# lucidrains/audiolm-pytorch

Measured on AMD Instinct MI355X. Metric: audio-tokens/sec fwd+bwd, CoarseTransformer d=1024 seq=2048, higher is better.
Workload: dtype bf16; 1 GPU; CoarseTransformer dim=1024 depth=6 heads=8 (MQA) num_coarse_quantizers=3 codebook=1024 semantic=500 residual_streams=4 flash_attn=True; per-GPU B=8, N=2048 (509 semantic + 512x3 coarse ids + eos/start); mask_prob=0.15; global_batch=8, seq_len=2048, parallelism=dp1, schedule=one hipGraph replay per step (captured fwd + bwd)

## Files before the change

audiolm-pytorch_amd/_lib.py:

```python
from __future__ import annotations

import ctypes
import os
from ctypes import c_float, c_int, c_longlong, c_ulonglong, c_void_p

_HERE = os.path.dirname(os.path.abspath(__file__))
LIB_PATH = os.environ.get('ALM_LIB_PATH') or os.path.join(_HERE, 'libaudiolm_hip.so')

_P, _I, _L, _F, _U = c_void_p, c_int, c_longlong, c_float, c_ulonglong

SIGNATURES = {
    'alm_gemm_bf16_nt': [_P, _P, _P, _P, _I, _I, _I, _L, _L, _L, _I, _I, _L, _L, _L, _L, _L, _L, _F, _I, _I, _P],
    'alm_gemm_bf16_nt_ws': [_P, _P, _P, _P, _I, _I, _I, _L, _L, _L, _I, _I, _L, _L, _L, _L, _L, _L, _F, _I, _I, _P, _L, _P],
    'alm_gemm_bf16_nt_inl': [_P, _P, _P, _P, _I, _I, _I, _L, _L, _L, _F, _I, _I, _I, _P, _L, _P],
    'alm_gemm_nt_plan': [_I, _I, _I, _I, _I, _P],
    'alm_gemm_nt_ws_bytes': [],
    'alm_gemm_splitk_slices': [_I, _I, _I, _I],
    'alm_gemm_splitk_ws_floats': [_I, _I, _I, _I],
    'alm_gemm_splitk_tile': [_I, _I, _I, _I],
    'alm_gemm_nt_tile_choice': [_I, _I, _I],
    'alm_gemm_tn_batched_plan': [_I, _I, _I, _I, _P],
    'alm_gemm_bf16_nt_splitk': [_P, _P, _P, _P, _I, _I, _I, _L, _L, _L, _I, _L, _L, _L, _F, _I, _P],
    'alm_gemm_bf16_tn_splitk': [_P, _P, _P, _P, _I, _I, _I, _L, _L, _L, _I, _L, _L, _L, _F, _I, _P],
    'alm_gemm_bf16_tn_batched': [_P, _P, _P, _P, _I, _I, _I, _L, _L, _L, _I, _I, _L, _L, _L, _L, _L, _L, _F, _I, _P],
    'alm_gemm_bf16_nt_group2': [_P, _P, _P, _I, _I, _I, _L, _L, _L, _P, _P, _P, _I, _I, _I, _L, _L, _L, _I, _P],
    'alm_gemm_bf16_nt_tile': [_P, _P, _P, _P, _I, _I, _I, _L, _L, _L, _F, _I, _I, _I, _P],
    'alm_transpose_bf16': [_P, _P, _I, _I, _L, _L, _I, _P],
    'alm_transpose_bf16_batched': [_P, _P, _I, _I, _L, _L, _I, _I, _L, _L, _P],
    'alm_pack_weights_multi': [_P, _I, _P],
    'alm_pack_weight': [_P, _I, _I, _L, _P, _L, _I, _I, _P, _L, _P],
    'alm_ln_partial_blocks': [_I],
    'alm_layernorm_fwd': [_P, _I, _L, _P, _P, _I, _L, _P, _L, _P, _P, _I, _I, _P],
    'alm_layernorm_bwd': [_P, _I, _L, _P, _I, _L, _P, _P, _P, _P, _L, _P, _I, _L, _P, _I, _I, _P],
    'alm_colsum': [_P, _I, _L, _I, _I, _P, _F, _I, _P, _P],
    'alm_colsum_chunks': [_I],
    'alm_colsum_partial': [_P, _L, _I, _I, _P, _P],
    'alm_geglu_fwd': [_P, _P, _L, _I, _P],
    'alm_geglu_bwd': [_P, _P, _P, _L, _I, _P],
    'alm_geglu_partial_blocks': [_I],
    'alm_geglu_ln_fwd': [_P, _L, _I, _P, _P, _L, _P, _P, _I, _I, _I, _P],
    'alm_geglu_ln_bwd': [_P, _L, _P, _L, _I, _P, _P, _P, _P, _P, _I, _I, _I, _P],
    'alm_mqa_attn_fwd': [_P, _L, _P, _L, _P, _L, _P, _P, _L, _P, _I, _I, _I, _I, _F, _F, _U, _P, _P],
    'alm_mqa_attn_bwd': [_P, _L, _P, _L, _P, _L, _P, _P, _L, _P, _P, _L, _P, _L, _P, _P, _L, _L, _P, _I, _I, _I, _I, _F, _F, _U, _P, _P],
    'alm_mqa_attn_bias_fwd': [_P, _L, _P, _L, _P, _L, _P, _P, _L, _P, _I, _I, _I, _I, _F, _P, _I, _P, _P, _P, _P, _F, _U, _P, _P],
    'alm_mqa_attn_bias_bwd': [_P, _L, _P, _L, _P, _L, _P, _P, _L, _P, _P, _L, _P, _L, _P, _P, _L, _L, _P, _I, _I, _I, _I, _F,
                              _P, _I, _P, _P, _P, _P, _P, _F, _U, _P, _P],
    'alm_attn_bias_part_rows': [_I, _I, _I],
    'alm_attn_bias_grad_reduce': [_P, _P, _I, _I, _I, _I, _F, _P],
    'alm_posmlp_in_fwd': [_P, _P, _P, _P, _P, _I, _I, _I, _P],
    'alm_posmlp_in_bwd_chunks': [_I],
    'alm_posmlp_in_bwd': [_P, _P, _P, _I, _I, _I, _P],
    'alm_silu_fwd': [_P, _P, _L, _P],
    'alm_silu_bwd': [_P, _P, _P, _L, _P],
    'alm_posmlp_out_fwd': [_P, _P, _P, _P, _P, _I, _I, _I, _F, _P],
    'alm_posmlp_out_bwd': [_P, _P, _P, _P, _P, _P, _I, _I, _I, _I, _F, _P],
    'alm_xattn_softmax_fwd': [_P, _L, _P, _P, _F, _P, _L, _P, _P, _P, _L, _I, _I, _I, _I, _I, _P],
    'alm_xattn_dbias': [_P, _L, _P, _L, _P, _P, _L, _I, _I, _I, _I, _P],
    'alm_xattn_combine': [_P, _L, _P, _P, _P, _L, _L, _I, _I, _P],
    'alm_xattn_softmax_bwd': [_P, _L, _P, _L, _P, _F, _P, _L, _I, _I, _I, _I, _P],
    'alm_xattn_delta': [_P, _L, _P, _L, _P, _I, _I, _I, _I, _P],
    'alm_value_residual_mix': [_P, _L, _P, _L, _P, _L, _L, _I, _P],
    'alm_kv_grad_pack': [_P, _P, _L, _I, _L, _P, _P, _L, _L, _I, _I, _P],
    'alm_forgetful_mask': [_P, _L, _P, _L, _I, _I, _I, _P],
    'alm_coarse_prepare': [_P, _L, _P, _L, _I, _I, _I, _L, _L, _L, _I, _I, _P, _P, _P, _P, _I, _P],
    'alm_semantic_prepare': [_P, _L, _I, _I, _L, _L, _P, _P, _I, _P],
    'alm_unique_consecutive_i64': [_P, _L, _I, _I, _I, _L, _L, _P, _L, _P, _P],
    'alm_fine_prepare': [_P, _L, _P, _L, _I, _I, _I, _L, _L, _I, _I, _I, _P, _P, _P],
    'alm_loss_combine': [_P, _P, _P, _P, _P, _P, _P, _P, _L, _L, _L, _L, _F, _F, _F, _F, _I, _L, _P, _P, _P],
    'alm_mqa_head_groups': [_I],
    'alm_mqa_bwd_parts': [_I, _I, _I],
    'alm_hc_coef_width': [_I],
    'alm_hc_partial_width': [_I, _I],
    'alm_hc_grads_width': [_I, _I],
    'alm_hc_partial_rows': [_I, _I, _I, _I, _L, _I],
    'alm_hc_fwd': [_P, _I, _I, _P, _L, _P, _P, _P, _P, _P, _P, _P, _P, _P, _P, _P, _L, _P, _L, _P, _P, _P, _P, _P, _I, _I, _I, _I, _I, _P],
    'alm_hc_bwd': [_P, _I, _I, _P, _L, _P, _L, _P, _L, _P, _P, _P, _P, _I, _P, _P, _P, _P, _P, _P, _P, _P, _P, _F, _P, _P, _L, _P, _P, _L, _P, _I, _I, _I, _I, _I, _P],
    'alm_hc_param_grads': [_P, _I, _P, _P, _P, _P, _I, _I, _P],
    'alm_hc_param_grads_batched': [_P, _P, _I, _P, _P, _P, _P, _P, _I, _I, _P],
    'alm_streams_expand': [_P, _P, _I, _I, _L, _P],
    'alm_streams_reduce': [_P, _P, _I, _I, _L, _P],
    'alm_residual_add': [_P, _P, _L, _P, _L, _I, _P],
    'alm_f32_to_bf16': [_P, _P, _P, _L, _L, _I, _P],
    'alm_add_f32': [_P, _P, _P, _L, _F, _P],
    'alm_embed_assemble': [_P, _P, _I, _P, _P, _P, _L, _I, _P, _P],
    'alm_embed_scatter_add': [_P, _P, _I, _P, _P, _P, _F, _L, _I, _P],
    'alm_embed_scatter_ws_floats': [_P, _I, _L, _I],
    'alm_embed_scatter_owned': [_P, _P, _I, _P, _P, _P, _F, _L, _I, _P, _P],
    'alm_gather_split_bf16': [_P, _L, _L, _P, _P, _P, _L, _L, _I, _P],
    'alm_gather_rows_bf16': [_P, _L, _P, _P, _L, _L, _I, _P],
    'alm_scatter_rows_bf16': [_P, _L, _P, _P, _L, _L, _I, _P],
    'alm_cross_entropy_fwd': [_P, _L, _P, _P, _P, _L, _I, _I, _P],
    'alm_cross_entropy_bwd': [_P, _L, _P, _P, _P, _P, _L, _L, _I, _I, _I, _P],
    'alm_reduce_sum': [_P, _L, _P, _F, _P],
    'alm_mqa_decode_attn': [_P, _L, _P, _L, _P, _L, _P, _L, _P, _L, _I, _I, _I, _I, _I, _F, _P, _I, _I, _I, _P, _P, _P, _P, _P, _P],
    'alm_opt_chunk_elems': [],
    'alm_opt_grad_sumsq': [_P, _I, _P, _I, _P, _P],
    'alm_opt_adam_step': [_P, _I, _P, _I, _F, _F, _F, _F, _I, _I, _P, _F, _P],
    'alm_opt_adam_pack_step': [_P, _I, _F, _F, _F, _F, _I, _I, _P, _F, _P],
    'alm_conv1d_packed_floats': [_I, _I, _I],
    'alm_conv1d_pack': [_P, _P, _I, _I, _I, _P],
    'alm_conv1d_causal': [_P, _P, _P, _P, _P, _I, _I, _I, _I, _I, _I, _I, _I, _I, _P],
    'alm_resunit_causal': [_P, _P, _P, _P, _P, _P, _I, _I, _I, _I, _I, _P],
    'alm_phase_interleave': [_P, _P, _I, _I, _I, _I, _P],
    'alm_rvq_decode': [_P, _L, _P, _P, _L, _I, _I, _I, _I, _P],
    'alm_rvq_padded_codes': [_I],
    'alm_rvq_padded_dim': [_I],
    'alm_rvq_pack': [_P, _P, _P, _I, _I, _I, _P],
    'alm_rvq_encode': [_P, _L, _P, _P, _P, _P, _L, _P, _L, _I, _I, _I, _I, _P],
    'alm_bct_to_btc': [_P, _P, _I, _I, _I, _P],
    'alm_conv1d_wgrad_chunk': [_I, _I],
    'alm_conv1d_wgrad_ws_floats': [_I, _I, _I, _I, _I],
    'alm_conv1d_dgrad': [_P, _P, _P, _P, _P, _I, _I, _I, _I, _I, _I, _I, _I, _P],
    'alm_conv1d_wgrad': [_P, _P, _P, _P, _P, _P, _L, _I, _I, _I, _I, _I, _I, _I, _I, _P],
    'alm_phase_deinterleave': [_P, _P, _I, _I, _I, _I, _P],
    'alm_resample_sinc': [_P, _L, _P, _L, _P, _I, _L, _L, _L, _I, _I, _I, _P],
    'alm_resample_sinc_bwd': [_P, _L, _P, _L, _P, _I, _L, _L, _L, _I, _I, _I, _P],
    'alm_hubert_conv0_chunks': [_L],
    'alm_hubert_conv0_stats': [_P, _L, _P, _P, _P, _I, _I, _L, _L, _I, _I, _F, _P],
    'alm_hubert_conv0_apply': [_P, _L, _P, _P, _P, _P, _P, _I, _I, _L, _L, _I, _I, _P],
# ... 94 lines not shown
```

audiolm-pytorch_amd/core.py:

```python
from __future__ import annotations

import os
import sys
from dataclasses import dataclass

import torch

from . import launchlist, ops, relpos, xattn

BF16, F32 = torch.bfloat16, torch.float32


@dataclass
class StackCfg:
    dim: int
    depth: int
    heads: int
    dim_head: int
    streams: int
    inner: int
    add_value_residual: bool
    grad_shrink_alpha: float
    residual_bf16: bool = False
    cross_attend: bool = False
# ... 475 lines not shown

    def _issue(self, stream, fn, tensors):
        ev = torch.cuda.Event()
        ev.record(self.main)
        for t in tensors:
            t.record_stream(stream)
        with torch.cuda.stream(stream):
            stream.wait_event(ev)
            return fn()

    def run(self, fn, *tensors):
        if not self.enabled:
            return fn()
        stream = self.streams[self.turn % len(self.streams)]
        self.turn += 1
        return self._issue(stream, fn, tensors)

    def run_after_all(self, fn, *tensors):
        if not self.enabled:
            return fn()
        s0 = self.streams[0]
        for s in self.streams[1:]:
            ev = torch.cuda.Event()
            ev.record(s)
            s0.wait_event(ev)
        return self._issue(s0, fn, tensors)

    def join(self):
        if self.enabled:
            for s in self.streams:
                ev = torch.cuda.Event()
                ev.record(s)
                self.main.wait_event(ev)


ASYNC_WGRAD = os.environ.get('ALM_ASYNC_WGRAD', '1') != '0'
QKV_GROUP = {'0': 0, '1': 1}.get(os.environ.get('ALM_QKV_GROUP', 'auto'), -1)
QKV_GROUP_MAX_M = 8192
ASYNC_KV = os.environ.get('ALM_ASYNC_KV', '0') != '0'
DEFER_WGRAD = os.environ.get('ALM_DEFER_WGRAD', '1') != '0'
DEFER_MAX_BYTES = int(float(os.environ.get('ALM_DEFER_MAX_GB', '24')) * (1 << 30))


def deferred_bytes(cfg, M):
    return cfg.depth * M * (2 * cfg.dim + 2 * cfg.inner_pad + cfg.heads * cfg.dim_head + 2 * cfg.dim_head) * 2
DEFER_GROUPS = max(1, int(os.environ.get('ALM_DEFER_GROUPS', '1')))
DP_DEFER_GROUPS = max(0, int(os.environ.get('ALM_DP_DEFER_GROUPS', '2')))
_DPGS = os.environ.get('ALM_DP_GROUP_SIZES', '').replace(' ', '').lower()
DP_GROUP_SIZES = None if _DPGS == '' else (() if _DPGS == 'even' else tuple(int(v) for v in _DPGS.split(',') if v))


def dp_group_sizes(L, ngroups):
    if DP_GROUP_SIZES is not None:
        return DP_GROUP_SIZES
    return (L - 1, 1) if (ngroups == 2 and L >= 3) else ()
DEFER_GROUP_SIZES = tuple(int(v) for v in os.environ.get('ALM_DEFER_GROUP_SIZES', '').replace(' ', '').split(',') if v)


def group_starts(L, ngroups, sizes=()):
    if sizes:
        if sum(sizes) != L or min(sizes) < 1:
            raise ValueError(f'ALM_DP_GROUP_SIZES={sizes}: the group sizes must be positive and sum to the depth {L}')
        starts, top = [], L
        for n in sizes:
            top -= n
            starts.append(top)
        return sorted(starts)
    gsz = (L + ngroups - 1) // ngroups
    return list(range(0, L, gsz))
HC_BATCH_FINISH = os.environ.get('ALM_HC_BATCH_FINISH', '1') != '0'
DEFER_SMALL_LATE = os.environ.get('ALM_DEFER_SMALL_LATE', '1') != '0'
_DEBUG_DEFER_GROUPS_CAPTURE = 1
MICRO_ASYNC_WGRAD = os.environ.get('ALM_MICRO_ASYNC_WGRAD', '0') != '0'
SIDE_STREAMS = max(1, int(os.environ.get('ALM_SIDE_STREAMS', '1')))


TRACE = None


def _vgrad_mode(acc, mixed):
    return 0 if acc is None else (1 if mixed else 2)


def ff_backward(cfg, W, prm, sv, dY, side, want_trace=False, du_out=None):
    M, D = dY.shape
    I, Ip, dev = cfg.inner, cfg.inner_pad, dY.device
    (_, W1T), (_, W2T) = W['w1'], W['w2']
    run = side.run if side is not None else (lambda fn, *t: fn())
    dHN = _empty((M, Ip), BF16, dev)
    fa = sv['alpha']
    ops.gemm_nt(dY, W2T, dHN, alpha=fa)
    if sv['keep'] is not None:
        dHN.mul_(sv['keep'])
    deferred = du_out is not None
    dW2 = None
    if not deferred:
        dW2 = _empty((D, I), F32, dev)
        HNs, dYs = sv['HN'], dY
        run(lambda: ops.gemm_tn_splitk(dYs, HNs[:, :I], dW2, alpha=fa), dYs, HNs, dW2)
    dU, dg3 = ops.geglu_ln_bwd(dHN, sv['U'], prm['ln3'], sv['mean3'], sv['rstd3'], I, Ip, du_out=du_out)
    dXN = _empty((M, D), BF16, dev)
    ops.gemm_nt(dU, W1T, dXN)
    dW1 = None
    if not deferred:
        dW1 = _empty((2 * I, D), F32, dev)
        XNs = sv['XN']
        run(lambda: ops.gemm_tn_splitk(dU.view(M, 2, Ip).permute(1, 0, 2)[:, :, :I], XNs, dW1.view(2, I, D)), dU, XNs, dW1)
    return (dXN, dW1, dg3, dW2, dHN, dU) if want_trace else (dXN, dW1, dg3, dW2)


def stack_backward(dhn, mask_u8, flat, cfg: StackCfg, cache: WeightCache, saved, on_layer_grads=None, bias=None, async_wgrad=True, dx_scale=1.0):
    B, N = saved['B'], saved['N']
    D, S, H, dh = cfg.dim, cfg.streams, cfg.heads, cfg.dim_head
    M = B * N
    I, Ip = cfg.inner, cfg.inner_pad
    dev = dhn.device
    ppl = params_per_layer(S, cfg.cross_attend)
    grads = [None] * len(flat)
    side = _SideStream(dev, ASYNC_WGRAD and async_wgrad)
    rdt = BF16 if (cfg.residual_bf16 and S > 1) else F32
    ctx = saved['ctx']
    brs = saved['branches']
    scale = float(dh) ** -0.5

    dxs, dgam = ops.layernorm_bwd(dhn, saved['xs'], saved['fmean'], saved['frstd'], flat[-1])
    grads[-1] = dgam
    multi = cfg.add_value_residual and cfg.depth > 1
    acc_v0 = ops._new_zeros((M, dh), dtype=F32, device=dev) if multi else None
    acc_vp0 = ops._new_zeros((B * ctx.m, dh), dtype=F32, device=dev) if (multi and cfg.prefix) else None
    acc_vc0 = ops._new_zeros((B * ctx.m, dh), dtype=F32, device=dev) if (multi and cfg.cross_attend) else None
    dctx = None
    dense = isinstance(bias, relpos.DenseBias)
    dtbl_part = ops.attn_bias_part(B, N, H, bias.tbl.shape[1], dev) if (bias is not None and not dense) else None
    ddense = torch.zeros_like(bias.tbl) if dense else None
    dR, bcast = dxs, S > 1
    dY = dbeta = None
    stk = saved.get('stk')
    bst = None
    if stk is not None:
        L = cfg.depth
        bst = dict(dYat=_empty((L, M, D), BF16, dev), dYff=_empty((L, M, D), BF16, dev), dU=_empty((L, M, 2 * Ip), BF16, dev),
                   dQ=_empty((L, M, H * dh), BF16, dev), dKV=_empty((L, M, 2 * dh), BF16, dev))

    def dy_slot(br):
        return None if bst is None else bst['dYat' if br['kind'] == 'attn' else 'dYff'][br['layer']]
    if S > 1:
        h = ops.hc_bwd(dxs, B, S, N, D, bcast=True, y_prev=brs[-1]['Y'], coef_prev=brs[-1]['coef'], r_dtype=rdt, dy_out=dy_slot(brs[-1]))
        dY, dbeta = h['dy'], h['dbeta']

    wg = None
    if bst is not None:
        L = cfg.depth
        ngroups = _DEBUG_DEFER_GROUPS_CAPTURE if (dev.type == 'cuda' and torch.cuda.is_current_stream_capturing()) else (
            DEFER_GROUPS if on_layer_grads is None else max(1, DP_DEFER_GROUPS))
        ngroups = min(ngroups, L)
        capturing = dev.type == 'cuda' and torch.cuda.is_current_stream_capturing()
        starts = group_starts(L, ngroups, () if capturing else (dp_group_sizes(L, ngroups) if on_layer_grads is not None else DEFER_GROUP_SIZES))
        ngroups = len(starts)
        on_group = getattr(on_layer_grads, 'on_group', None)
        group_buffer = getattr(on_layer_grads, 'group_buffer', None)
        wg = True
        wshape = dict(dW1=(2, I, D), dW2=(1, D, I), dWo=(1, D, H * dh), dWq=(1, H * dh, D), dWkv=(1, 2 * dh, D))
        hc_n_ = 7 if S > 1 else 0
        wslot = dict(dWq=hc_n_ + 1, dWkv=hc_n_ + 2, dWo=hc_n_ + 3, dW1=(hc_n_ + 4) + hc_n_ + 1, dW2=(hc_n_ + 4) + hc_n_ + 3)

        big_kinds, small_kinds = ('dW1', 'dW2'), ('dWo', 'dWq', 'dWkv')
        late = DEFER_SMALL_LATE and ngroups > 1
        handed = set()

        def group_outputs(l0, l1, kinds, late_kinds):
            views = None
            if group_buffer is not None:
                views = group_buffer(l0, l1, [wslot[k] for k in kinds], [wslot[k] for k in late_kinds],
                                     [wslot[k] for k in small_kinds] if (late and not late_kinds) else [])
            if views is not None:
                return {k: v.view(-1, *wshape[k]) for k, v in zip(tuple(kinds) + tuple(late_kinds), views)}
            out = {k: _empty((l1 - l0,) + wshape[k], F32, dev) for k in kinds}
            out.update({k: _empty((L,) + wshape[k], F32, dev) for k in late_kinds})
            return out

        def launch_group(l0):
            l1 = ([s_ for s_ in starts if s_ > l0] + [L])[0]
            last = l0 == 0
            kinds = big_kinds if late else big_kinds + small_kinds
            late_kinds = small_kinds if (late and last) else ()
            wgg = group_outputs(l0, l1, kinds, late_kinds)
            operands = dict(dW1=lambda a, b: (bst['dU'][a:b].view(b - a, M, 2, Ip).permute(0, 2, 1, 3)[..., :I], stk['XNff'][a:b].unsqueeze(1)),
                            dW2=lambda a, b: (bst['dYff'][a:b].unsqueeze(1), stk['HN'][a:b][..., :I].unsqueeze(1)),
                            dWo=lambda a, b: (bst['dYat'][a:b].unsqueeze(1), stk['AO'][a:b].unsqueeze(1)),
                            dWq=lambda a, b: (bst['dQ'][a:b].unsqueeze(1), stk['XNat'][a:b].unsqueeze(1)),
                            dWkv=lambda a, b: (bst['dKV'][a:b].unsqueeze(1), stk['Xat'][a:b].unsqueeze(1)))
            jobs = [operands[k](l0, l1) + (wgg[k],) for k in kinds] + [operands[k](0, L) + (wgg[k],) for k in late_kinds]
            for At, Bt, C in jobs:
                if ngroups > 1 or on_layer_grads is not None:
                    side.run(lambda At=At, Bt=Bt, C=C: ops.gemm_tn_batched(At, Bt, C), At, Bt, C)
                else:
                    ops.gemm_tn_batched(At, Bt, C)
            for k in kinds:
                for l in range(l0, l1):
                    g_ = wgg[k][l - l0]
                    grads[l * ppl + wslot[k]] = g_.view(2 * I, D) if k == 'dW1' else g_[0]
            for k in late_kinds:
                for l in range(L):
                    grads[l * ppl + wslot[k]] = wgg[k][l, 0]
            if on_layer_grads is not None:
                layers = list(range((L if late_kinds else l1) - 1, l0 - 1, -1))
                per_layer = []
                for l in layers:
                    gl = [g if (l * ppl + j) not in handed else None for j, g in enumerate(grads[l * ppl:(l + 1) * ppl])]
                    handed.update(l * ppl + j for j, g in enumerate(gl) if g is not None)
                    per_layer.append(gl)
                live = [g for gl in per_layer for g in gl if g is not None]
                if on_group is not None:
                    side.run_after_all(lambda: on_group(layers, per_layer), *live)
                else:
                    def hand_off():
                        for l, gl in zip(layers, per_layer):
                            on_layer_grads(l, gl)
                    side.run_after_all(hand_off, *live)

    hc_pending = []

    def finish_hc():
        if not hc_pending:
            return
        for (first_, ip_, _, rec_), g_ in zip(hc_pending, ops.hc_param_grads_batched([t[2] for t in hc_pending], S, D)):
            for j, k in enumerate(HC_KEYS):
                grads[first_ + j] = g_[k]
            grads[ip_] = g_['ln']
            if rec_ is not None:
                rec_['hc_grads'] = dict(g_)
        hc_pending.clear()

    def add_ctx(g):
        nonlocal dctx
        dctx = g if dctx is None else ops.add_f32(dctx, g)

    LW, LW_layer = None, -1
    for bi in reversed(range(len(brs))):
        sv = brs[bi]
        kind, l, first = sv['kind'], sv['layer'], sv['first']
        if l != LW_layer:
            branches = _split_layer(flat[l * ppl:(l + 1) * ppl], S, cfg.cross_attend)
            LW, LW_layer = layer_weights(cache, l, branches, I, Ip), l
            prms = {k: (d, f) for k, d, f in branches}
        prm = prms[kind][0]
        hc_n = 7 if S > 1 else 0
        ip = first + hc_n
        if S == 1:
            dY = ops.f32_to_bf16(dR, out=dy_slot(sv))
        extra = None
        W = LW[kind]
        if kind == 'ff':
            dXN, dW1, dg3, dW2, dHN, dU = ff_backward(cfg, W, prm, sv, dY, side, want_trace=True, du_out=bst['dU'][l] if bst is not None else None)
            grads[ip + 1], grads[ip + 2], grads[ip + 3] = dW1, dg3, dW2
            rec = dict(dY=dY, dHN=dHN, dU=dU, dXN=dXN, dW1=dW1, dg3=dg3, dW2=dW2) if TRACE is not None else None
        elif kind == 'cross':
            (_, WqT), (_, WkvT), (_, WoT) = W['wq'], W['wkv'], W['wo']
            m = ctx.m
            dAO = _empty((M, H * dh), BF16, dev)
            oa = sv['oalpha']
            dYs = dY if sv['okeep'] is None else dY * sv['okeep']
            ops.gemm_nt(dYs, WoT, dAO, alpha=oa)
            dWo = _empty((D, H * dh), F32, dev)
            AOs = sv['AO']
            side.run(lambda: ops.gemm_tn_splitk(dYs, AOs, dWo, alpha=oa), dYs, AOs, dWo)
            nd = xattn.attn_delta(sv['AO'], dAO, B, N, H, dh)
            dQ, dke, dve = xattn.extra_attn_bwd(sv['Q'], dAO, sv['xs'], nd, B, N, H, dh, scale)
            dnull = torch.stack((dke[:, 0].sum(0), dve[:, 0].sum(0))).reshape(2, 1, dh)
            dkv32 = torch.cat((dke[:, 1:].reshape(B * m, dh), dve[:, 1:].reshape(B * m, dh)), dim=1).contiguous()
            dKVc = ops.kv_grad_pack(dkv32, acc_vc0, _vgrad_mode(acc_vc0, sv['cmixed']), dh)
            dXN = _empty((M, D), BF16, dev)
            ops.gemm_nt(dQ, WqT, dXN)
            dWq = _empty((H * dh, D), F32, dev)
            XNs = sv['XN']
            side.run(lambda: ops.gemm_tn_splitk(dQ, XNs, dWq), dQ, XNs, dWq)
            dCN = _empty((B * m, cfg.dim_context), BF16, dev)
            ops.gemm_nt(dKVc, WkvT, dCN)
            dWkv = _empty((2 * dh, cfg.dim_context), F32, dev)
            CNs = sv['CN']
            side.run(lambda: ops.gemm_tn_splitk(dKVc, CNs, dWkv), dKVc, CNs, dWkv)
            dc, dgc = ops.layernorm_bwd(dCN, ctx.x, sv['cmean'], sv['crstd'], prm['ctx_ln'])
            add_ctx(dc)
            grads[ip + 1], grads[ip + 2], grads[ip + 3], grads[ip + 4], grads[ip + 5] = dgc, dnull, dWq, dWkv, dWo
            rec = dict(dY=dY) if TRACE is not None else None
        else:
            (_, WqT), (_, WkvT), (_, WoT) = W['wq'], W['wkv'], W['wo']
            dAO = _empty((M, H * dh), BF16, dev)
            oa = sv['oalpha']
            dYs = dY if sv['okeep'] is None else dY * sv['okeep']
            ops.gemm_nt(dYs, WoT, dAO, alpha=oa)
            dWo = dWq = dWkv = None
            if bst is None:
                dWo = _empty((D, H * dh), F32, dev)
                AOs = sv['AO']
                side.run(lambda: ops.gemm_tn_splitk(dYs, AOs, dWo, alpha=oa), dYs, AOs, dWo)
            pd, dseed, dseed_dev = sv['drop']
            KV = sv['KV']
            dense_pre = None
            if dense:
                nd = xattn.attn_delta(sv['AO'], dAO, B, N, H, dh)
                mpre = ctx.m if sv['pre'] is not None else 0
                dbl = torch.empty((H, N, mpre + N), dtype=F32, device=dev)
                dQ, dke, dve = xattn.extra_attn_bwd(sv['Q'], dAO, sv['dense'], nd, B, N, H, dh, scale, dbias=dbl)
                ddense += dbl[:, :, mpre:]
                if mpre:
                    dense_pre = (dke[:, :mpre], dve[:, :mpre])
                    dke, dve = dke[:, mpre:], dve[:, mpre:]
                dkv32 = torch.cat((dke.reshape(M, dh), dve.reshape(M, dh)), dim=1).contiguous()
            else:
                dQ, dkv32 = ops.mqa_attn_bwd(sv['Q'], KV[:, :dh], sv['V'], mask_u8, sv['AO'], sv['LSE'], dAO, B, N, H, dh, bias=bias, dtbl_part=dtbl_part,
                                             dropout_p=pd, seed=dseed, dq_out=bst['dQ'][l] if bst is not None else None, seed_dev=dseed_dev)
            dKV = ops.kv_grad_pack(dkv32, acc_v0, _vgrad_mode(acc_v0, sv['mixed']), dh, out=bst['dKV'][l] if bst is not None else None)
            dKVp = None
            pre = sv['pre']
            if pre is not None:
                m = ctx.m
                if dense_pre is not None:
                    dke, dve = dense_pre
                else:
                    nd = xattn.attn_delta(sv['AO'], dAO, B, N, H, dh)
                    dQ, dke, dve = xattn.extra_attn_bwd(sv['Q'], dAO, pre['xs'], nd, B, N, H, dh, scale, dq=dQ)
                dkvp32 = torch.cat((dke.reshape(B * m, dh), dve.reshape(B * m, dh)), dim=1).contiguous()
                dKVp = ops.kv_grad_pack(dkvp32, acc_vp0, _vgrad_mode(acc_vp0, pre['pmixed']), dh)
                dcp = _empty((B * m, D), F32, dev)
                ops.gemm_nt(dKVp, WkvT, dcp)
                add_ctx(dcp)
            dXN = _empty((M, D), BF16, dev)
            extra = _empty((M, D), BF16, dev)
            ops.gemm_nt_group2(dQ, WqT, dXN, dKV, WkvT, extra)
            if bst is None:
                dWq = _empty((H * dh, D), F32, dev)
                XNs = sv['XN']
                side.run(lambda: ops.gemm_tn_splitk(dQ, XNs, dWq), dQ, XNs, dWq)
                dWkv = _empty((2 * dh, D), F32, dev)
                Xs, cx = sv['X'], (ctx.x if dKVp is not None else None)

                def wkv_grad():
                    ops.gemm_tn_splitk(dKV, Xs, dWkv)
                    if dKVp is not None:
                        ops.gemm_tn_splitk(dKVp, cx, dWkv, accumulate=True)
                side.run(wkv_grad, *[t for t in (dKV, Xs, dWkv, dKVp, cx) if t is not None])
            grads[ip + 1], grads[ip + 2], grads[ip + 3] = dWq, dWkv, dWo
            rec = dict(dY=dY, dAO=dAO, dQ=dQ, dkv32=dkv32, dKV=dKV, dXN=dXN, extra=extra, dWq=dWq, dWkv=dWkv, dWo=dWo) if TRACE is not None else None

        prev = brs[bi - 1] if bi > 0 else None
        if S > 1:
            py, pc = (prev['Y'], prev['coef']) if prev is not None else (None, None)
            h = ops.hc_bwd(dR, B, S, N, D, bcast=bcast, dxn=dXN, extra=extra, mean=sv['mean'], rstd=sv['rstd'], ln_gamma=prm['ln'], R=sv['R'],
                           coef=sv['coef'], dbeta=dbeta, hc=prm['hc'], y_prev=py, coef_prev=pc, r_bcast=sv['r_bcast'], sum_only=prev is None,
                           r_dtype=rdt, dsum_scale=dx_scale if prev is None else 1.0, dy_out=dy_slot(prev) if prev is not None else None,
                           defer_grads=wg is not None and HC_BATCH_FINISH)
            if rec is not None:
                rec.update(kind=kind, layer=l, dR_in=dR, dR_in_bcast=bcast, dbeta_in=dbeta, dR_out=h['dsum'] if prev is None else h['dR'], sum_only=prev is None,
                           dY_prev=h['dy'], dbeta_prev=h['dbeta'], hc_grads=dict(h['grads']) if h['grads'] is not None else None)
                TRACE.append(rec)
            dR, dY, dbeta, bcast = (h['dsum'] if prev is None else h['dR']), h['dy'], h['dbeta'], False
            if h['grads'] is None:
                hc_pending.append((first, ip, h['part'], rec))
            else:
                for j, k in enumerate(HC_KEYS):
                    grads[first + j] = h['grads'][k]
                grads[ip] = h['grads']['ln']
        else:
            dX, dgl = ops.layernorm_bwd(dXN, sv['R'], sv['mean'], sv['rstd'], prm['ln'], extra=extra)
            if rec is not None:
                rec.update(kind=kind, layer=l, dR_in=dR, dX=dX, dln=dgl)
                TRACE.append(rec)
            dR = ops.add_f32(dR, dX, dx_scale if prev is None else 1.0)
            grads[ip] = dgl
        sv.clear()
        if wg is not None and (prev is None or prev['layer'] != l) and l in starts:
            finish_hc()
            launch_group(l)
        if on_layer_grads is not None and wg is None and (prev is None or prev['layer'] != l):
            base = l * ppl
            side.run_after_all(lambda: on_layer_grads(l, grads[base:base + ppl]), *[g for g in grads[base:base + ppl] if g is not None])

    finish_hc()
    dx = dR.view(B, N, D)
    dtbl = ddense if dense else (ops.attn_bias_grad_reduce(dtbl_part, B, N, H) if bias is not None else None)
    side.join()
    return dx, grads, dtbl, dctx


_MICRO_STREAMS = {}


def _micro_stream(dev):
    key = (dev.type, dev.index)
    if key not in _MICRO_STREAMS:
        _MICRO_STREAMS[key] = torch.cuda.Stream(device=dev)
    return _MICRO_STREAMS[key]


def _halves(t, h):
    return (None, None) if t is None else (t[:h], t[h:])


class TransformerStackFn(torch.autograd.Function):

    @staticmethod
    def forward(ctx, x, mask_u8, cfg, cache, opts, bias, tbl, context, *flat):
        hooks = opts.get('hook')
        need = bool(opts.get('grad', True)) and (any(t.requires_grad for t in flat) or x.requires_grad or (tbl is not None and tbl.requires_grad)
                                                 or (context is not None and context.requires_grad))
        xin = x.detach().contiguous().to(F32)
        bias = bias.detached() if bias is not None else None
        flat_d = flat
        B = xin.shape[0]
        cx = None
        if context is not None:
            m = context.shape[1]
            cm = opts.get('context_mask')
            cm = None if cm is None else cm.to(torch.bool).contiguous().view(torch.uint8)
            cx = Context(context.detach().to(BF16).reshape(B * m, -1).contiguous(), cm, B, m)
        ctx.ctx_meta = None if context is None else (context.shape, context.dtype)
        micro = int(opts.get('micro', 1))
        if micro == 2 and (B % 2 or B < 2 or opts.get('kv_out') is not None or opts.get('decode') is not None or hooks is not None):
            micro = 1
        ctx.micro = micro
        dseed = None
        if float(opts.get('attn_dropout', 0.)) > 0. and xin.is_cuda and torch.cuda.is_current_stream_capturing():
            seed_state = graph_seed_state(xin.device)
            seed_state.add_(2 * cfg.depth)
            dseed = (0, seed_state.clone())
        if micro == 1:
            defer = DEFER_WGRAD and (hooks is None or DP_DEFER_GROUPS > 0)
            plan = None
            if (launchlist.ENABLED and hooks is None and cx is None and opts.get('kv_out') is None and opts.get('decode') is None and TRACE is None
                    and float(opts.get('ff_dropout', 0.)) == 0. and float(opts.get('attn_dropout', 0.)) == 0. and not isinstance(bias, relpos.DenseBias)
                    and xin.is_cuda and not torch.cuda.is_current_stream_capturing()):
                plan = launchlist.plan_for(sys.modules[__name__], xin, mask_u8, cfg, need, bias, len(flat_d), defer, cfg.grad_shrink_alpha)
            if plan is not None:
                hn, saved = launchlist.forward(sys.modules[__name__], plan, xin, mask_u8, flat_d, cfg, cache, need, bias, defer)
            else:
                hn, saved = stack_forward(xin, mask_u8, flat_d, cfg, cache, need, bias, kv_out=opts.get('kv_out'), decode=opts.get('decode'), ctx=cx,
                                          ff_dropout=float(opts.get('ff_dropout', 0.)), attn_dropout=float(opts.get('attn_dropout', 0.)),
                                          defer_wgrad=defer, drop_seed=dseed)
        else:
            S, ppl, h = cfg.streams, params_per_layer(cfg.streams, cfg.cross_attend), B // 2
            for l in range(cfg.depth):
                layer_weights(cache, l, _split_layer(flat_d[l * ppl:(l + 1) * ppl], S, cfg.cross_attend), cfg.inner, cfg.inner_pad)
            cur, s2 = torch.cuda.current_stream(xin.device), _micro_stream(xin.device)
            (xa, xb), (ma, mb) = _halves(xin, h), _halves(mask_u8, h)
            ca = cb = None
            if cx is not None:
                (cma, cmb) = _halves(cx.mask, h)
                ca, cb = Context(cx.x[:h * cx.m], cma, h, cx.m), Context(cx.x[h * cx.m:], cmb, B - h, cx.m)
            s2.wait_stream(cur)
            adp = float(opts.get('attn_dropout', 0.))
            hna, sva = stack_forward(xa, ma, flat_d, cfg, cache, need, bias, ctx=ca, ff_dropout=float(opts.get('ff_dropout', 0.)), attn_dropout=adp, drop_seed=dseed)
            xb.record_stream(s2)
            with torch.cuda.stream(s2):
                hnb, svb = stack_forward(xb, mb, flat_d, cfg, cache, need, bias, ctx=cb, ff_dropout=float(opts.get('ff_dropout', 0.)), attn_dropout=adp,
                                         drop_seed=None if dseed is None else (cfg.depth, dseed[1]))
            cur.wait_stream(s2)
            hnb.record_stream(cur)
            hn = torch.cat((hna, hnb), dim=0)
            saved = (sva, svb)
        ctx.saved, ctx.cfg, ctx.cache, ctx.mask, ctx.hooks, ctx.bias = saved, cfg, cache, mask_u8, hooks, bias
        ctx.flat = flat
# ... 46 lines not shown
```

audiolm-pytorch_amd/csrc/gemm.hip:

```cpp
#include <algorithm>
#include <cstdlib>
#include <type_traits>

#include "common.hpp"
#include "../../include/audiolm_hip.h"

#ifndef ALM_GEMM_AUX_A
#define ALM_GEMM_AUX_A 0
#endif
#ifndef ALM_GEMM_AUX_B
#define ALM_GEMM_AUX_B 0
#endif

namespace {

constexpr int BK = 64;
constexpr unsigned OOB = 0x80000000u;

typedef __attribute__((address_space(3))) void lds_void;

struct GemmParams {
    const bf16_t* A;
    const bf16_t* B;
    void* C;
    const float* bias;
    int M, N, K;
    long long lda, ldb, ldc;
    int nb2;
    long long sA1, sA2, sB1, sB2, sC1, sC2;
    float alpha;
    int accumulate;
    int ksplit;
    long long sCk;
    int raster;
    int nsl;
    int nbt = 0;
    int plimit = 0;
    int group_m = 8;
    int nt_store = 0;
    float* inl_ws = nullptr;
    unsigned* inl_cnt = nullptr;
    int inl_slices = 0;
};

__device__ __forceinline__ int grouped_tile(int bid, int tiles_m, int tiles_n, int g) {
    const bool rows = g > 0;
    const int ga = rows ? g : -g;
    const int t_in = rows ? tiles_n : tiles_m, t_gr = rows ? tiles_m : tiles_n;
    const int per_group = ga * t_in;
    const int group = bid / per_group, rem = bid % per_group;
    const int first = group * ga;
    const int gsz = min(t_gr - first, ga);
    const int a = first + rem % gsz, b = rem / gsz;
    return rows ? (a | (b << 16)) : (b | (a << 16));
}

template <int BM, int BN, int WM, int WN, int TM, int TNB, bool OUT_F32>
__device__ __forceinline__ void gemm_epilogue(const GemmParams& p, f32x16 (&acc)[TM][TNB], unsigned char* slabs, long long coff0, int m0, int n0,
                                              int wave, int wr, int wc, int lane, int lr, int lh) {
    {
        constexpr int ES = OUT_F32 ? 4 : 2;
        constexpr int WCOLS = 32 * TNB;
        constexpr int ROWB = WCOLS * ES;
        constexpr int NCH = ROWB / 16;
        constexpr int SLAB = 32 * ROWB;
        unsigned char* Cb = reinterpret_cast<unsigned char*>(p.C) + coff0 * ES;
        const bool fast = !p.accumulate && ((p.ldc * ES) & 15) == 0 && ((uintptr_t)Cb & 15) == 0 && (p.N % (16 / ES)) == 0;
        if (fast) {
            unsigned char* slab = slabs + wave * SLAB;
            const int ncol0 = n0 + wc * (BN / WN);
#pragma unroll
            for (int i = 0; i < TM; ++i) {
                const int mrow0 = m0 + wr * (BM / WM) + i * 32;
#pragma unroll
                for (int j = 0; j < TNB; ++j)
#pragma unroll
                    for (int g = 0; g < 4; ++g) {
                        const int c0 = j * 32 + 8 * g + 4 * lh;
                        float v[4];
#pragma unroll
                        for (int c = 0; c < 4; ++c) {
                            v[c] = acc[i][j][4 * g + c] * p.alpha;
                            if (p.bias && ncol0 + c0 + c < p.N) v[c] += p.bias[ncol0 + c0 + c];
                        }
                        if (OUT_F32) {
                            const int ch = c0 / 4;
                            *reinterpret_cast<float4*>(slab + lr * ROWB + ((ch ^ (lr & (NCH - 1))) << 4)) = make_float4(v[0], v[1], v[2], v[3]);
// ... 784 lines not shown
#pragma unroll
        for (int i = 0; i < TM; ++i)
#pragma unroll
            for (int j = 0; j < TNB; ++j) acc[i][j] = __builtin_amdgcn_mfma_f32_32x32x16_bf16(f.b[j], f.a[i], acc[i][j], 0, 0, 0);
    };
    constexpr int NMF = TM * TNB;
    constexpr int NRD = (TNMODE ? 2 : 1) * (TM + TNB);

    const int nk = (Krem + BK - 1) / BK;
    Frags F0, F1, F2, F3;

    stage(0, smem);
    if (nk > 1) { stage_a(1, smem + STAGE); wait_vmcnt<8>(); } else wait_vmcnt<0>();
    __builtin_amdgcn_s_barrier();
    load_frags(smem, 0, F0);
    GPROBE_T(0);

    auto kstep = [&](unsigned char* __restrict__ cur, unsigned char* __restrict__ nxt, int kt, auto m2c, auto m1c) {
        constexpr bool MORE2 = decltype(m2c)::value, MORE1 = decltype(m1c)::value;
        if (MORE1) stage_b(kt + 1, nxt);
        load_frags(cur, 1, F1);
        mfma_all(F0);
#pragma unroll
        for (int q = 0; q < NMF / 2; ++q) {
            __builtin_amdgcn_sched_group_barrier(0x008, 2, 0);
            if (MORE1) __builtin_amdgcn_sched_group_barrier(0x010, 1, 0);
            __builtin_amdgcn_sched_group_barrier(0x100, (NRD + NMF / 2 - 1) / (NMF / 2), 0);
        }
        __builtin_amdgcn_sched_barrier(0);
        GPROBE_T(1);
        load_frags(cur, 2, F2);
        mfma_all(F1);
        load_frags(cur, 3, F3);
        mfma_all(F2);
#pragma unroll
        for (int g = 0; g < 2; ++g)
#pragma unroll
            for (int q = 0; q < NMF / 2; ++q) {
                __builtin_amdgcn_sched_group_barrier(0x008, 2, 0);
                __builtin_amdgcn_sched_group_barrier(0x100, (NRD + NMF / 2 - 1) / (NMF / 2), 0);
            }
        __builtin_amdgcn_sched_barrier(0);
        GPROBE_T(2);
        if (MORE1) {
            asm volatile("s_waitcnt vmcnt(0) lgkmcnt(0)" ::: "memory");
            __builtin_amdgcn_s_barrier();
            __builtin_amdgcn_sched_barrier(0);
        }
        GPROBE_T(3);
        if (MORE2) stage_a(kt + 2, cur);
        if (MORE1) load_frags(nxt, 0, F0);
        mfma_all(F3);
#pragma unroll
        for (int q = 0; q < NMF / 2; ++q) {
            __builtin_amdgcn_sched_group_barrier(0x008, 2, 0);
            if (MORE2) __builtin_amdgcn_sched_group_barrier(0x010, 1, 0);
            if (MORE1) __builtin_amdgcn_sched_group_barrier(0x100, (NRD + NMF / 2 - 1) / (NMF / 2), 0);
        }
        __builtin_amdgcn_sched_barrier(0);
        GPROBE_T(4);
    };
    using T = std::true_type;
    using F = std::false_type;
    int kt = 0;
#pragma unroll 1
    for (; kt + 2 < nk; ++kt) kstep(smem + (kt & 1) * STAGE, smem + ((kt & 1) ^ 1) * STAGE, kt, T{}, T{});
    if (kt + 1 < nk) { kstep(smem + (kt & 1) * STAGE, smem + ((kt & 1) ^ 1) * STAGE, kt, F{}, T{}); ++kt; }
    kstep(smem + (kt & 1) * STAGE, smem + ((kt & 1) ^ 1) * STAGE, kt, F{}, F{});
    __syncthreads();

    constexpr int ES = OUT_F32 ? 4 : 2;
    static_assert(NW * 32 * (32 * TNB * ES) <= 2 * STAGE, "epilogue slab");
    const long long coff0 = z1 * p.sC1 + z2 * p.sC2 + (p.ksplit > 0 ? zs * p.sCk : 0);
    gemm_epilogue<BM, BN, WM, WN, TM, TNB, OUT_F32>(p, acc, smem, coff0, m0, n0, wave, wr, wc, lane, lr, lh);
    GPROBE_T(6);
    GPROBE_FLUSH((blockIdx.x + gridDim.x * (blockIdx.y + gridDim.y * blockIdx.z)) * 4 + wave);
}

__global__ __launch_bounds__(256) void splitk_reduce_kernel(const float* __restrict__ ws, int splits, long long mn, long long slice_stride, int N,
                                                            float* __restrict__ C, long long ldc, long long sC, int accumulate,
                                                            int nb2 = 0x40000000, long long sC1 = 0) {
    ws += (long long)blockIdx.y * mn;
    C += (long long)(blockIdx.y / nb2) * sC1 + (long long)(blockIdx.y % nb2) * sC;
    const bool vec = (N & 3) == 0 && (ldc & 3) == 0 && ((uintptr_t)C & 15) == 0 && (mn & 3) == 0 && (slice_stride & 3) == 0;
    if (vec) {
        const long long mn4 = mn >> 2;
        for (long long i = (long long)blockIdx.x * 256 + threadIdx.x; i < mn4; i += (long long)gridDim.x * 256) {
            float4 s = make_float4(0.f, 0.f, 0.f, 0.f);
            for (int z = 0; z < splits; ++z) {
                const float4 v = *reinterpret_cast<const float4*>(ws + (long long)z * slice_stride + i * 4);
                s.x += v.x; s.y += v.y; s.z += v.z; s.w += v.w;
            }
            const long long e = i * 4, m = e / N, n = e % N;
            float4* c = reinterpret_cast<float4*>(C + m * ldc + n);
            if (accumulate) { const float4 w = *c; s.x += w.x; s.y += w.y; s.z += w.z; s.w += w.w; }
            *c = s;
        }
        return;
    }
    for (long long i = (long long)blockIdx.x * 256 + threadIdx.x; i < mn; i += (long long)gridDim.x * 256) {
        float s = 0.f;
        for (int z = 0; z < splits; ++z) s += ws[(long long)z * slice_stride + i];
        const long long m = i / N, n = i % N;
        float* c = C + m * ldc + n;
        *c = accumulate ? *c + s : s;
    }
}

__global__ __launch_bounds__(256) void transpose_bf16_kernel(const bf16_t* __restrict__ src, bf16_t* __restrict__ dst, int rows, int cols,
                                                             long long ld_src, long long ld_dst, int rows_pad, long long bs_src,
                                                             long long bs_dst) {
    __shared__ bf16_t tile[64][66];
    src += (long long)blockIdx.z * bs_src;
    dst += (long long)blockIdx.z * bs_dst;
    const int r0 = blockIdx.y * 64, c0 = blockIdx.x * 64;
    const int tx = threadIdx.x & 63, ty = threadIdx.x >> 6;
    for (int i = ty; i < 64; i += 4) {
        const int r = r0 + i, c = c0 + tx;
        tile[i][tx] = (r < rows && c < cols) ? src[(long long)r * ld_src + c] : (bf16_t)0;
    }
    __syncthreads();
    for (int i = ty; i < 64; i += 4) {
        const int c = c0 + i, r = r0 + tx;
        if (c < cols && r < rows_pad) dst[(long long)c * ld_dst + r] = tile[tx][i];
    }
}

__global__ __launch_bounds__(256) void pack_weight_kernel(const float* __restrict__ src, int rows, int cols, long long ld_src,
                                                          bf16_t* __restrict__ dst, long long ld_dst, int rows_pad, int cols_pad,
                                                          bf16_t* __restrict__ dstT, long long ld_dstT) {
    __shared__ bf16_t tile[64][66];
    const int r0 = blockIdx.y * 64, c0 = blockIdx.x * 64;
    const int tx = threadIdx.x & 63, ty = threadIdx.x >> 6;
    for (int i = ty; i < 64; i += 4) {
        const int r = r0 + i, c = c0 + tx;
        const bf16_t v = (r < rows && c < cols) ? f2bf(src[(long long)r * ld_src + c]) : (bf16_t)0;
        tile[i][tx] = v;
        if (dst && r < rows_pad && c < cols_pad) dst[(long long)r * ld_dst + c] = v;
    }
    if (!dstT) return;
    __syncthreads();
    for (int i = ty; i < 64; i += 4) {
        const int c = c0 + i, r = r0 + tx;
        if (c < cols_pad && r < rows_pad) dstT[(long long)c * ld_dstT + r] = tile[tx][i];
    }
}

struct PackJobs {
    AlmPackJob job[8];
    int tile_end[8];
    int njobs;
};
__global__ __launch_bounds__(256) void pack_weights_multi_kernel(PackJobs pj) {
    __shared__ bf16_t tile[64][66];
    int j = 0;
    while (j + 1 < pj.njobs && (int)blockIdx.x >= pj.tile_end[j]) ++j;
    const AlmPackJob& q = pj.job[j];
    const int local = blockIdx.x - (j ? pj.tile_end[j - 1] : 0);
    const int tcols = (q.cols_pad + 63) / 64;
    const int r0 = (local / tcols) * 64, c0 = (local % tcols) * 64;
    const int tx = threadIdx.x & 63, ty = threadIdx.x >> 6;
    bf16_t* dst = reinterpret_cast<bf16_t*>(q.dst);
    bf16_t* dstT = reinterpret_cast<bf16_t*>(q.dstT);
    for (int i = ty; i < 64; i += 4) {
        const int r = r0 + i, c = c0 + tx;
        const bf16_t v = (r < q.rows && c < q.cols) ? f2bf(q.src[(long long)r * q.ld_src + c]) : (bf16_t)0;
        tile[i][tx] = v;
        if (dst && r < q.rows_pad && c < q.cols_pad) dst[(long long)r * q.ld_dst + c] = v;
    }
    if (!dstT) return;
    __syncthreads();
    for (int i = ty; i < 64; i += 4) {
        const int c = c0 + i, r = r0 + tx;
        if (c < q.cols_pad && r < q.rows_pad) dstT[(long long)c * q.ld_dstT + r] = tile[tx][i];
    }
}

struct PackJobs2 {
    AlmPackJob job[8];
    int tile_end[8];
    int njobs;
};
__global__ __launch_bounds__(256) void pack_weights_multi2_kernel(PackJobs2 pj) {
    __shared__ uint32_t tile[64][65];
    int j = 0;
    while (j + 1 < pj.njobs && (int)blockIdx.x >= pj.tile_end[j]) ++j;
    const AlmPackJob& q = pj.job[j];
    const int local = blockIdx.x - (j ? pj.tile_end[j - 1] : 0);
    const int tcols = (q.cols_pad + 127) / 128;
// ... 269 lines not shown
    }
    return best;
}

int nt_launch_ws(const GemmParams& p0, int ny, int out_f32, int force_slices, void* ws, long long ws_bytes, hipStream_t st) {
    NtPlan pl = nt_plan(p0.M, p0.N, p0.K, ny);
    if (force_slices > 0) {
        const long long t256 = (long long)((p0.M + 255) / 256) * ((p0.N + 255) / 256) * ny;
        if (p0.M < 256 || p0.N < 256 || t256 > 1024) return ALM_ERR_UNSUPPORTED;
        pl = NtPlan{13, force_slices};
    }
    if (force_slices == 0 && (pl.tile != 13 || pl.slices < 2)) return launch_gemm<false>(p0, ny, 1, out_f32, 0, st);
    const long long tiles = (long long)((p0.M + 255) / 256) * ((p0.N + 255) / 256) * ny;
    if (pl.slices == 1) return launch_gemm<false>(p0, ny, 1, out_f32, 13, st, false);
    const long long need = INL_CNT_BYTES + tiles * pl.slices * INL_SLAB_BYTES;
    if (!ws || ws_bytes < need || ((uintptr_t)ws & 15)) {
        if (force_slices > 0) return ALM_ERR_BAD_ARG;
        return launch_gemm<false>(p0, ny, 1, out_f32, 0, st);
    }
    GemmParams p = p0;
    const int ksteps = (p.K + BK - 1) / BK;
    p.ksplit = (ksteps + pl.slices - 1) / pl.slices * BK;
    p.sCk = 0;
    p.inl_slices = (p.K + p.ksplit - 1) / p.ksplit;
    if (p.inl_slices < 2) return launch_gemm<false>(p0, ny, 1, out_f32, 13, st, false);
    p.inl_cnt = reinterpret_cast<unsigned*>(ws);
    p.inl_ws = reinterpret_cast<float*>(reinterpret_cast<unsigned char*>(ws) + INL_CNT_BYTES);
    p.group_m = pick_group(p, 13);
    return out_f32 ? launch_stag_inl<true>(p, ny, st) : launch_stag_inl<false>(p, ny, st);
}

struct SplitPlan { int tile, slices; };

int pick_raster(int M, int N, int nb, int tile) {
    const int bm = tile >= 2 ? 256 : 128;
    const int tmm = (M + bm - 1) / bm, tnn = (N + bm - 1) / bm;
    const int P = (tmm >= tnn ? tmm : tnn) * nb;
    return (P % 8 == 0 || P >= 20) ? 1 : 0;
}
SplitPlan splitk_plan(int M, int N, int K, int nb) {
    SplitPlan best{1, 1};
    double best_t = 1e30;
    for (int tile = 1; tile <= 2; ++tile) {
        if (tile == 2 && (M < 256 || N < 256)) continue;
        const int bm = tile == 2 ? 256 : 128;
        const double tiles = (double)((M + bm - 1) / bm) * ((N + bm - 1) / bm) * nb;
        const double slots = tile == 2 ? 256.0 : 512.0;
        const double us_per_kstep = tile == 2 ? 2.0 : 1.25;
        for (int s = 1; s <= 64; ++s) {
            if (s > 1 && (K + s - 1) / s < 256) break;
            const int kc = ((K + s - 1) / s + BK - 1) / BK * BK;
            const int nsl = (K + kc - 1) / kc;
            if (nsl != s) continue;
            const double waves = ceil(tiles * s / slots);
            double t = waves * ((kc / BK) * us_per_kstep + 3.0);
            if (s > 1) t += (double)s * M * N * nb * 8.0 / 4.0e6 + 3.0;
            if (t < best_t) { best_t = t; best = SplitPlan{tile == 2 ? 13 : 1, s}; }
        }
    }
    return best;
}

struct HybridPlan { int panels_a, m_major, off, slices_b; };
HybridPlan hybrid_plan(int M, int N, int K, int nb) {
    static const int off_switch = [] { const char* e = getenv("ALM_GEMM_HYBRID"); return e ? atoi(e) : 1; }();
    HybridPlan none{0, 0, 0, 0};
    if (!off_switch || M < 256 || N < 256 || K < 4096) return none;
    const int tm = (M + 255) / 256, tn = (N + 255) / 256;
    const int m_major = tm >= tn, tmaj = m_major ? tm : tn, Q = m_major ? tn : tm;
    const int P = tmaj * nb, total = P * Q;
    if (total <= 256) return none;
    const int panels_a = (total / 256) * 256 / Q;
    const int rem = P - panels_a;
    if (panels_a * Q % 256 != 0 || rem <= 0 || rem >= tmaj || rem * Q > 64) return none;
    const int off = (tmaj - rem) * 256;
    int s = 256 / (rem * Q);
    const int ksteps = (K + BK - 1) / BK;
    while (s > 1 && ksteps / s < 8) --s;
    if (s < 2) return none;
    return HybridPlan{panels_a, m_major, off, s};
}

int splitk_fixed(const bf16_t* At, const bf16_t* Bt, float* C, float* ws, int M, int N, int K, long long lda, long long ldb, long long ldc, int slices,
                 float alpha, int accumulate, hipStream_t st) {
    int kc = (K + slices - 1) / slices;
    kc = (kc + BK - 1) / BK * BK;
    const int nsl = (K + kc - 1) / kc;
    const long long mn = (long long)M * N;
    GemmParams p{At, Bt, ws, nullptr, M, N, K, lda, ldb, (long long)N, 1, 0, 0, 0, 0, 0, mn, alpha, 0, kc, mn, 0, nsl, 1};
    int rc = launch_gemm<true>(p, 1, nsl, 1, 13, st);
    if (rc) return rc;
    const int grid = (int)((mn + 255) / 256 < 2048 ? (mn + 255) / 256 : 2048);
    hipLaunchKernelGGL(splitk_reduce_kernel, dim3(grid, 1), dim3(256), 0, st, (const float*)ws, nsl, mn, mn, N, C, ldc, 0LL, accumulate);
    return 0;
}

}

extern "C" int alm_gemm_bf16_nt(const void* A, const void* B, void* C, const float* bias, int M, int N, int K, long long lda,
                                long long ldb, long long ldc, int nb1, int nb2, long long sA1, long long sA2, long long sB1,
                                long long sB2, long long sC1, long long sC2, float alpha, int out_f32, int accumulate, void* stream) {
    if (M <= 0 || N <= 0 || nb1 <= 0 || nb2 <= 0) return 0;
    if (K <= 0 || (K & 7) || (lda & 7) || (ldb & 7) || ((uintptr_t)A & 15) || ((uintptr_t)B & 15)) return ALM_ERR_BAD_ARG;
    if (((sA1 | sA2 | sB1 | sB2) & 7) != 0) return ALM_ERR_BAD_ARG;
    if (view_too_big(384, lda) || view_too_big(256, ldb)) return ALM_ERR_UNSUPPORTED;
    GemmParams p{(const bf16_t*)A, (const bf16_t*)B, C, bias, M, N, K, lda, ldb, ldc, nb2, sA1, sA2, sB1, sB2, sC1, sC2, alpha, accumulate, 0, 0, 0, 1};
    int rc = launch_gemm<false>(p, nb1 * nb2, 1, out_f32, 0, (hipStream_t)stream);
    if (rc) return rc;
    ALM_LAUNCH_CHECK();
    return 0;
}

extern "C" int alm_gemm_bf16_nt_ws(const void* A, const void* B, void* C, const float* bias, int M, int N, int K, long long lda, long long ldb, long long ldc,
                                   int nb1, int nb2, long long sA1, long long sA2, long long sB1, long long sB2, long long sC1, long long sC2, float alpha,
                                   int out_f32, int accumulate, void* ws, long long ws_bytes, void* stream) {
    if (M <= 0 || N <= 0 || nb1 <= 0 || nb2 <= 0) return 0;
    if (K <= 0 || (K & 7) || (lda & 7) || (ldb & 7) || ((uintptr_t)A & 15) || ((uintptr_t)B & 15)) return ALM_ERR_BAD_ARG;
    if (((sA1 | sA2 | sB1 | sB2) & 7) != 0) return ALM_ERR_BAD_ARG;
    if (view_too_big(384, lda) || view_too_big(256, ldb)) return ALM_ERR_UNSUPPORTED;
    GemmParams p{(const bf16_t*)A, (const bf16_t*)B, C, bias, M, N, K, lda, ldb, ldc, nb2, sA1, sA2, sB1, sB2, sC1, sC2, alpha, accumulate, 0, 0, 0, 1};
    int rc = nt_launch_ws(p, nb1 * nb2, out_f32, 0, ws, ws_bytes, (hipStream_t)stream);
    if (rc) return rc;
    ALM_LAUNCH_CHECK();
    return 0;
}

extern "C" int alm_gemm_bf16_nt_inl(const void* A, const void* B, void* C, const float* bias, int M, int N, int K, long long lda, long long ldb, long long ldc,
                                    float alpha, int out_f32, int accumulate, int slices, void* ws, long long ws_bytes, void* stream) {
    if (M <= 0 || N <= 0) return 0;
    if (K <= 0 || (K & 7) || (lda & 7) || (ldb & 7) || ((uintptr_t)A & 15) || ((uintptr_t)B & 15) || slices < 1 || slices > 16) return ALM_ERR_BAD_ARG;
    if (view_too_big(384, lda) || view_too_big(256, ldb)) return ALM_ERR_UNSUPPORTED;
    GemmParams p{(const bf16_t*)A, (const bf16_t*)B, C, bias, M, N, K, lda, ldb, ldc, 1, 0, 0, 0, 0, 0, 0, alpha, accumulate, 0, 0, 0, 1};
    int rc = nt_launch_ws(p, 1, out_f32, slices, ws, ws_bytes, (hipStream_t)stream);
    if (rc) return rc;
    ALM_LAUNCH_CHECK();
    return 0;
}

extern "C" int alm_gemm_nt_plan(int M, int N, int K, int nb, int with_ws, int* plan) {
    nb = nb < 1 ? 1 : nb;
    NtPlan pl = with_ws ? nt_plan(M, N, K, nb) : NtPlan{pick_tile(M, N, nb, 0, false), 1};
    int tile = pl.tile;
    const long long t128 = (long long)((M + 127) / 128) * ((N + 127) / 128) * nb;
    static const int ring_on = [] { const char* e = getenv("ALM_GEMM_RING"); return e ? atoi(e) : 1; }();
    if (tile == 1 && ring_on && K >= 256 && t128 <= 256) tile = 16;
    const long long bm = tile == 11 ? 384 : (tile == 17 ? 320 : (tile == 13 ? 256 : 128)), bn = tile == 1 || tile == 16 ? 128 : 256;
    const long long wgs = ((M + bm - 1) / bm) * ((N + bn - 1) / bn) * nb * pl.slices;
    if (plan) {
        plan[0] = tile; plan[1] = pl.slices;
        plan[2] = pl.slices > 1 ? (int)(INL_CNT_BYTES + (wgs * INL_SLAB_BYTES)) : 0;
        plan[3] = (int)wgs;
    }
    return 0;
}

extern "C" int alm_gemm_nt_ws_bytes(void) { return (int)(INL_CNT_BYTES + 256 * INL_SLAB_BYTES); }

extern "C" int alm_gemm_bf16_nt_group2(const void* A0, const void* B0, void* C0, int M0, int N0, int K0, long long lda0, long long ldb0, long long ldc0,
                                       const void* A1, const void* B1, void* C1, int M1, int N1, int K1, long long lda1, long long ldb1, long long ldc1,
                                       int out_f32, void* stream) {
    static const int on = [] { const char* e = getenv("ALM_GEMM_GROUP2"); return e ? atoi(e) : 1; }();
    hipStream_t st = (hipStream_t)stream;
    auto bad = [](const void* A, const void* B, int K, long long lda, long long ldb) {
        return K <= 0 || (K & 7) || (lda & 7) || (ldb & 7) || ((uintptr_t)A & 15) || ((uintptr_t)B & 15);
    };
    if (M0 <= 0 || N0 <= 0 || M1 <= 0 || N1 <= 0) {
        int rc = alm_gemm_bf16_nt(A0, B0, C0, nullptr, M0, N0, K0, lda0, ldb0, ldc0, 1, 1, 0, 0, 0, 0, 0, 0, 1.f, out_f32, 0, stream);
        if (rc) return rc;
        return alm_gemm_bf16_nt(A1, B1, C1, nullptr, M1, N1, K1, lda1, ldb1, ldc1, 1, 1, 0, 0, 0, 0, 0, 0, 1.f, out_f32, 0, stream);
    }
    if (bad(A0, B0, K0, lda0, ldb0) || bad(A1, B1, K1, lda1, ldb1)) return ALM_ERR_BAD_ARG;
    if (view_too_big(384, lda0) || view_too_big(256, ldb0) || view_too_big(384, lda1) || view_too_big(256, ldb1)) return ALM_ERR_UNSUPPORTED;
    int t0 = pick_tile(M0, N0, 1, 0, false), t1 = pick_tile(M1, N1, 1, 0, false);
    static const int grp_big = [] { const char* e = getenv("ALM_GEMM_GROUP2_BIG"); return e ? atoi(e) : 0; }();
    if (grp_big && t0 == 1 && t1 == 1 && M0 >= 256 && N0 >= 256 && M1 >= 256 && N1 >= 256) {
        const long long a = (long long)((M0 + 255) / 256) * ((N0 + 255) / 256), b = (long long)((M1 + 255) / 256) * ((N1 + 255) / 256);
        if (a + b >= 192 && a + b <= 256 && (a & 7) == 0) t0 = t1 = 13;
// ... 36 lines not shown
    GemmParams p{(const bf16_t*)A, (const bf16_t*)B, C, bias, M, N, K, lda, ldb, ldc, 1, 0, 0, 0, 0, 0, 0, alpha, accumulate, 0, 0, 0, 1};
    int rc = launch_gemm<false>(p, 1, 1, out_f32, tile, (hipStream_t)stream, false);
    if (rc) return rc;
    ALM_LAUNCH_CHECK();
    return 0;
}

extern "C" int alm_gemm_splitk_slices(int M, int N, int K, int nb) { return splitk_plan(M, N, K, nb < 1 ? 1 : nb).slices; }

extern "C" int alm_gemm_splitk_tile(int M, int N, int K, int nb) { return splitk_plan(M, N, K, nb < 1 ? 1 : nb).tile; }

extern "C" int alm_gemm_nt_tile_choice(int M, int N, int nb) { return pick_tile(M, N, nb < 1 ? 1 : nb, 0, false); }

extern "C" int alm_gemm_tn_batched_plan(int M, int N, int K, int nb, int* plan) {
    nb = nb < 1 ? 1 : nb;
    const HybridPlan hy = hybrid_plan(M, N, K, nb);
    if (hy.panels_a > 0) {
        if (plan) { plan[0] = hy.panels_a; plan[1] = hy.slices_b; plan[2] = hy.off; plan[3] = hy.m_major; }
        return 2;
    }
    const SplitPlan pl = splitk_plan(M, N, K, nb);
    if (plan) { plan[0] = pl.tile; plan[1] = pl.slices; plan[2] = 0; plan[3] = 0; }
    return pl.slices > 1 ? 1 : 0;
}

extern "C" int alm_gemm_splitk_ws_floats(int M, int N, int K, int nb) {
    nb = nb < 1 ? 1 : nb;
    const SplitPlan pl = splitk_plan(M, N, K, nb);
    long long fl = pl.slices > 1 ? (long long)pl.slices * nb * M * N : 0;
    const HybridPlan hy = hybrid_plan(M, N, K, nb);
    if (hy.panels_a > 0) {
        const long long m2 = hy.m_major ? M - hy.off : M, n2 = hy.m_major ? N : N - hy.off;
        const long long f2 = (long long)hy.slices_b * m2 * n2;
        if (f2 > fl) fl = f2;
    }
    return fl > 0x7fffffffLL ? -1 : (int)fl;
}

static int splitk_common(bool tn, const void* A, const void* B, float* C, float* ws, int M, int N, int K, long long lda, long long ldb,
                         long long ldc, int nb, long long sA, long long sB, long long sC, float alpha, int accumulate, hipStream_t st) {
    const SplitPlan pl = splitk_plan(M, N, K, nb);
    if (pl.slices <= 1) {
        GemmParams p{(const bf16_t*)A, (const bf16_t*)B, C, nullptr, M, N, K, lda, ldb, ldc, nb, 0, sA, 0, sB, 0, sC, alpha, accumulate, 0, 0, pick_raster(M, N, nb, pl.tile), 1};
        return tn ? launch_gemm<true>(p, nb, 1, 1, pl.tile, st) : launch_gemm<false>(p, nb, 1, 1, pl.tile, st);
    }
    if (!ws) return ALM_ERR_BAD_ARG;
    int kc = (K + pl.slices - 1) / pl.slices;
    kc = (kc + BK - 1) / BK * BK;
    const int nsl = (K + kc - 1) / kc;
    const long long mn = (long long)M * N;
    GemmParams p{(const bf16_t*)A, (const bf16_t*)B, ws, nullptr, M, N, K, lda, ldb, (long long)N, nb, 0, sA, 0, sB, 0, mn, alpha, 0, kc, mn * nb, pick_raster(M, N, nb, pl.tile), nsl};
    int rc = tn ? launch_gemm<true>(p, nb, nsl, 1, pl.tile, st) : launch_gemm<false>(p, nb, nsl, 1, pl.tile, st);
    if (rc) return rc;
    const int grid = (int)((mn + 255) / 256 < 2048 ? (mn + 255) / 256 : 2048);
    hipLaunchKernelGGL(splitk_reduce_kernel, dim3(grid, nb), dim3(256), 0, st, (const float*)ws, nsl, mn, mn * nb, N, C, ldc, sC, accumulate);
    return 0;
}


extern "C" int alm_gemm_bf16_nt_splitk(const void* A, const void* B, float* C, float* ws, int M, int N, int K, long long lda, long long ldb,
                                       long long ldc, int nb, long long sA, long long sB, long long sC, float alpha, int accumulate,
                                       void* stream) {
    if (M <= 0 || N <= 0 || nb <= 0) return 0;
    if (K <= 0 || (K & 7) || (lda & 7) || (ldb & 7) || ((sA | sB) & 7) || ((uintptr_t)A & 15) || ((uintptr_t)B & 15)) return ALM_ERR_BAD_ARG;
    if (view_too_big(256, lda) || view_too_big(256, ldb)) return ALM_ERR_UNSUPPORTED;
    int rc = splitk_common(false, A, B, C, ws, M, N, K, lda, ldb, ldc, nb, sA, sB, sC, alpha, accumulate, (hipStream_t)stream);
    if (rc) return rc;
    ALM_LAUNCH_CHECK();
    return 0;
}

extern "C" int alm_gemm_bf16_tn_splitk(const void* At, const void* Bt, float* C, float* ws, int M, int N, int K, long long lda,
                                       long long ldb, long long ldc, int nb, long long sA, long long sB, long long sC, float alpha,
                                       int accumulate, void* stream) {
    if (M <= 0 || N <= 0 || nb <= 0) return 0;
    if (K <= 0 || (lda & 7) || (ldb & 7) || ((sA | sB) & 7) || ((uintptr_t)At & 15) || ((uintptr_t)Bt & 15)) return ALM_ERR_BAD_ARG;
    if (view_too_big(K, lda) || view_too_big(K, ldb)) return ALM_ERR_UNSUPPORTED;
    int rc = splitk_common(true, At, Bt, C, ws, M, N, K, lda, ldb, ldc, nb, sA, sB, sC, alpha, accumulate, (hipStream_t)stream);
    if (rc) return rc;
    ALM_LAUNCH_CHECK();
    return 0;
}

extern "C" int alm_gemm_bf16_tn_batched(const void* At, const void* Bt, float* C, float* ws, int M, int N, int K, long long lda, long long ldb,
                                        long long ldc, int nb1, int nb2, long long sA1, long long sA2, long long sB1, long long sB2, long long sC1,
                                        long long sC2, float alpha, int accumulate, void* stream) {
    if (M <= 0 || N <= 0 || nb1 <= 0 || nb2 <= 0) return 0;
    if (K <= 0 || (lda & 7) || (ldb & 7) || ((sA1 | sA2 | sB1 | sB2) & 7) || ((uintptr_t)At & 15) || ((uintptr_t)Bt & 15)) return ALM_ERR_BAD_ARG;
    if (view_too_big(K, lda) || view_too_big(K, ldb)) return ALM_ERR_UNSUPPORTED;
    hipStream_t st = (hipStream_t)stream;
    const int nb = nb1 * nb2;
    const SplitPlan pl = splitk_plan(M, N, K, nb);
    int rc;
    const HybridPlan hy = hybrid_plan(M, N, K, nb);
    if (hy.panels_a > 0) {
        static const int raster_a = [] { const char* e = getenv("ALM_GEMM_HYBRID_RASTER"); return e ? atoi(e) : 2; }();
        GemmParams pa{(const bf16_t*)At, (const bf16_t*)Bt, C, nullptr, M, N, K, lda, ldb, ldc, nb2, sA1, sA2, sB1, sB2, sC1, sC2, alpha, accumulate, 0, 0,
                      (hy.panels_a % 8 == 0 && raster_a == 2) ? 2 : 1, 1, nb, hy.panels_a};
        rc = launch_gemm<true>(pa, nb, 1, 1, 13, st, true, true);
        if (rc) return rc;
        const long long zA = (long long)(nb1 - 1) * sA1 + (long long)(nb2 - 1) * sA2, zB = (long long)(nb1 - 1) * sB1 + (long long)(nb2 - 1) * sB2;
        const long long zC = (long long)(nb1 - 1) * sC1 + (long long)(nb2 - 1) * sC2;
        const bf16_t* A2 = (const bf16_t*)At + zA + (hy.m_major ? hy.off : 0);
        const bf16_t* B2 = (const bf16_t*)Bt + zB + (hy.m_major ? 0 : hy.off);
        float* C2 = C + zC + (hy.m_major ? (long long)hy.off * ldc : hy.off);
        const int M2 = hy.m_major ? M - hy.off : M, N2 = hy.m_major ? N : N - hy.off;
        if (!ws) return ALM_ERR_BAD_ARG;
        rc = splitk_fixed(A2, B2, C2, ws, M2, N2, K, lda, ldb, ldc, hy.slices_b, alpha, accumulate, st);
        if (rc) return rc;
        ALM_LAUNCH_CHECK();
        return 0;
    }
    if (pl.slices <= 1) {
        GemmParams p{(const bf16_t*)At, (const bf16_t*)Bt, C, nullptr, M, N, K, lda, ldb, ldc, nb2, sA1, sA2, sB1, sB2, sC1, sC2, alpha, accumulate, 0, 0,
                     pick_raster(M, N, nb, pl.tile), 1, nb};
        rc = launch_gemm<true>(p, nb, 1, 1, pl.tile, st);
    } else {
        if (!ws) return ALM_ERR_BAD_ARG;
        int kc = (K + pl.slices - 1) / pl.slices;
        kc = (kc + BK - 1) / BK * BK;
        const int nsl = (K + kc - 1) / kc;
        const long long mn = (long long)M * N;
        GemmParams p{(const bf16_t*)At, (const bf16_t*)Bt, ws, nullptr, M, N, K, lda, ldb, (long long)N, nb2, sA1, sA2, sB1, sB2, mn * nb2, mn, alpha, 0, kc, mn * nb,
                     pick_raster(M, N, nb, pl.tile), nsl, nb};
        rc = launch_gemm<true>(p, nb, nsl, 1, pl.tile, st);
        if (rc) return rc;
        const int grid = (int)((mn + 255) / 256 < 2048 ? (mn + 255) / 256 : 2048);
        hipLaunchKernelGGL(splitk_reduce_kernel, dim3(grid, nb), dim3(256), 0, st, (const float*)ws, nsl, mn, mn * nb, N, C, ldc, sC2, accumulate, nb2, sC1);
    }
    if (rc) return rc;
    ALM_LAUNCH_CHECK();
    return 0;
}

extern "C" int alm_transpose_bf16(const void* src, void* dst, int rows, int cols, long long ld_src, long long ld_dst, int rows_pad,
                                  void* stream) {
    if (rows <= 0 || cols <= 0) return 0;
    if (rows_pad < rows || ld_dst < rows_pad) return ALM_ERR_BAD_ARG;
    dim3 grid((cols + 63) / 64, (rows_pad + 63) / 64);
    hipLaunchKernelGGL(transpose_bf16_kernel, grid, dim3(256), 0, (hipStream_t)stream, (const bf16_t*)src, (bf16_t*)dst, rows, cols, ld_src,
                       ld_dst, rows_pad, 0LL, 0LL);
    ALM_LAUNCH_CHECK();
    return 0;
}

extern "C" int alm_transpose_bf16_batched(const void* src, void* dst, int rows, int cols, long long ld_src, long long ld_dst, int rows_pad, int nb,
                                          long long bs_src, long long bs_dst, void* stream) {
    if (rows <= 0 || cols <= 0 || nb <= 0) return 0;
    if (rows_pad < rows || ld_dst < rows_pad || nb > 65535) return ALM_ERR_BAD_ARG;
    dim3 grid((cols + 63) / 64, (rows_pad + 63) / 64, nb);
    hipLaunchKernelGGL(transpose_bf16_kernel, grid, dim3(256), 0, (hipStream_t)stream, (const bf16_t*)src, (bf16_t*)dst, rows, cols, ld_src,
                       ld_dst, rows_pad, bs_src, bs_dst);
    ALM_LAUNCH_CHECK();
    return 0;
}

static int pack3_launch(const AlmPackJob* jobs, int njobs, hipStream_t st) {
    PackJobs3 pj{};
    int total = 0;
    for (int j = 0; j < njobs; ++j) {
        pj.job[j] = jobs[j];
        total += ((jobs[j].cols_pad + 127) / 128) * ((jobs[j].rows_pad + 63) / 64);
        pj.tile_end[j] = total;
    }
    pj.njobs = njobs;
    hipLaunchKernelGGL(pack_weights_multi3_kernel, dim3(total), dim3(256), 0, st, pj);
    return 0;
}

extern "C" int alm_pack_weights_multi(const AlmPackJob* jobs, int njobs, void* stream) {
    if (njobs <= 0) return 0;
    if (!jobs) return ALM_ERR_BAD_ARG;
    static const int wide_on = [] { const char* e = getenv("ALM_PACK_WIDE"); return e ? atoi(e) : 1; }();
    bool vec = true, wide = wide_on != 0;
    for (int j = 0; j < njobs; ++j) {
        const AlmPackJob& q = jobs[j];
        if (q.rows <= 0 || q.cols <= 0 || q.rows_pad < q.rows || q.cols_pad < q.cols) return ALM_ERR_BAD_ARG;
        if ((q.dst && q.ld_dst < q.cols_pad) || (q.dstT && q.ld_dstT < q.rows_pad)) return ALM_ERR_BAD_ARG;
        vec = vec && !((q.ld_src | q.ld_dst | q.ld_dstT | q.rows_pad | q.cols_pad) & 1) && !((uintptr_t)q.src & 7) && !((uintptr_t)q.dst & 3) &&
              !((uintptr_t)q.dstT & 3);
        wide = wide && q.cols >= 4 && !((q.ld_dst | q.ld_dstT | q.rows_pad | q.cols_pad) & 7) && !((uintptr_t)q.src & 3) && !((uintptr_t)q.dst & 15) && !((uintptr_t)q.dstT & 15);
    }
    hipStream_t st = (hipStream_t)stream;
    if (wide) {
        for (int j0 = 0; j0 < njobs; j0 += PACK3_JOBS) {
            int rc = pack3_launch(jobs + j0, std::min(PACK3_JOBS, njobs - j0), st);
            if (rc) return rc;
        }
        ALM_LAUNCH_CHECK();
        return 0;
    }
    for (int j0 = 0; j0 < njobs; j0 += 8) {
        const int nj = std::min(8, njobs - j0);
        if (vec) {
            PackJobs2 pj{};
            int total = 0;
            for (int j = 0; j < nj; ++j) {
                pj.job[j] = jobs[j0 + j];
                total += ((jobs[j0 + j].cols_pad + 127) / 128) * ((jobs[j0 + j].rows_pad + 63) / 64);
                pj.tile_end[j] = total;
            }
            pj.njobs = nj;
            hipLaunchKernelGGL(pack_weights_multi2_kernel, dim3(total), dim3(256), 0, st, pj);
        } else {
            PackJobs pj{};
            int total = 0;
            for (int j = 0; j < nj; ++j) {
                const AlmPackJob& q = jobs[j0 + j];
                pj.job[j] = q;
                total += ((q.cols_pad + 63) / 64) * ((q.rows_pad + 63) / 64);
                pj.tile_end[j] = total;
            }
            pj.njobs = nj;
            hipLaunchKernelGGL(pack_weights_multi_kernel, dim3(total), dim3(256), 0, st, pj);
        }
// ... 24 lines not shown
```

audiolm-pytorch_amd/csrc/launchlist.hip:

```cpp
#include <hip/hip_runtime.h>
#include <stdint.h>
#include <string.h>

#include <utility>
#include <vector>

#include "../../include/audiolm_hip.h"

namespace {

template <class T> struct Slot;
template <> struct Slot<int> { static int get(uint64_t v) { return (int)(int64_t)v; } };
template <> struct Slot<long long> { static long long get(uint64_t v) { return (long long)v; } };
template <> struct Slot<unsigned long long> { static unsigned long long get(uint64_t v) { return (unsigned long long)v; } };
template <> struct Slot<float> {
    static float get(uint64_t v) {
        uint32_t u = (uint32_t)v;
        float f;
        memcpy(&f, &u, 4);
        return f;
    }
};
template <class T> struct Slot<T*> { static T* get(uint64_t v) { return (T*)(uintptr_t)v; } };

template <class... A, size_t... I> int invoke(int (*f)(A...), const uint64_t* a, std::index_sequence<I...>) { return f(Slot<A>::get(a[I])...); }
template <class... A> int call_packed(int (*f)(A...), const uint64_t* a) { return invoke(f, a, std::index_sequence_for<A...>{}); }
template <class... A> constexpr int arity(int (*)(A...)) { return (int)sizeof...(A); }

struct Op {
    const char* name;
    int nargs;
    int (*thunk)(const uint64_t*);
};

#define ALM_OP(fn) {#fn, arity(fn), [](const uint64_t* a) -> int { return call_packed(fn, a); }}

__global__ __launch_bounds__(256) void zero_bytes_kernel(unsigned char* __restrict__ p, long long n) {
    const uintptr_t a = reinterpret_cast<uintptr_t>(p);
    const long long head = (long long)((16 - (a & 15)) & 15) < n ? (long long)((16 - (a & 15)) & 15) : n;
    const long long nvec = (n - head) / 16;
    uint4* v = reinterpret_cast<uint4*>(p + head);
    for (long long i = (long long)blockIdx.x * 256 + threadIdx.x; i < nvec; i += (long long)gridDim.x * 256) v[i] = make_uint4(0, 0, 0, 0);
    if (blockIdx.x == 0) {
        if ((long long)threadIdx.x < head) p[threadIdx.x] = 0;
        const long long tail0 = head + nvec * 16;
        if (tail0 + threadIdx.x < n && threadIdx.x < 16) p[tail0 + threadIdx.x] = 0;
    }
}

const Op OPS[] = {
    ALM_OP(alm_memset_zero),
    ALM_OP(alm_gemm_bf16_nt),
    ALM_OP(alm_gemm_bf16_nt_ws),
    ALM_OP(alm_gemm_bf16_nt_group2),
    ALM_OP(alm_gemm_bf16_nt_splitk),
    ALM_OP(alm_gemm_bf16_tn_splitk),
    ALM_OP(alm_gemm_bf16_tn_batched),
    ALM_OP(alm_layernorm_fwd),
    ALM_OP(alm_layernorm_bwd),
    ALM_OP(alm_colsum),
    ALM_OP(alm_colsum_partial),
    ALM_OP(alm_geglu_ln_fwd),
    ALM_OP(alm_geglu_ln_bwd),
    ALM_OP(alm_mqa_attn_fwd),
    ALM_OP(alm_mqa_attn_bwd),
    ALM_OP(alm_mqa_attn_bias_fwd),
    ALM_OP(alm_mqa_attn_bias_bwd),
    ALM_OP(alm_attn_bias_grad_reduce),
    ALM_OP(alm_value_residual_mix),
    ALM_OP(alm_kv_grad_pack),
    ALM_OP(alm_hc_fwd),
    ALM_OP(alm_hc_bwd),
    ALM_OP(alm_hc_param_grads),
    ALM_OP(alm_hc_param_grads_batched),
    ALM_OP(alm_streams_expand),
    ALM_OP(alm_streams_reduce),
    ALM_OP(alm_residual_add),
    ALM_OP(alm_f32_to_bf16),
    ALM_OP(alm_add_f32),
};
constexpr int NOPS = (int)(sizeof(OPS) / sizeof(OPS[0]));

}

extern "C" {

int alm_memset_zero(void* ptr, long long bytes, void* stream) {
    if (bytes < 0 || (bytes > 0 && ptr == nullptr)) return ALM_ERR_BAD_ARG;
    if (bytes == 0) return 0;
    const long long chunks = (bytes + 15) / 16 + 1;
    const long long blocks = (chunks + 255) / 256;
    hipLaunchKernelGGL(zero_bytes_kernel, dim3((unsigned)(blocks < 65535 * 16 ? blocks : 65535 * 16)), dim3(256), 0, (hipStream_t)stream,
                       reinterpret_cast<unsigned char*>(ptr), bytes);
    return (int)hipGetLastError();
}

int alm_list_op_id(const char* name) {
    if (name == nullptr) return -1;
    for (int i = 0; i < NOPS; ++i)
        if (strcmp(OPS[i].name, name) == 0) return i;
    return -1;
}

int alm_list_op_nargs(int op) { return (op >= 0 && op < NOPS) ? OPS[op].nargs : -1; }

int alm_list_run(const AlmListEntry* entries, int n, const unsigned long long* slots, const unsigned short* reloc, int nslots, const unsigned long long* bases,
                 int nbases, void* stream, int* failed_at) {
    if (failed_at) *failed_at = -1;
    if (n < 0 || nslots < 0 || nbases < 0 || (n > 0 && entries == nullptr) || (nslots > 0 && (slots == nullptr || reloc == nullptr)) || (nbases > 0 && bases == nullptr))
        return ALM_ERR_BAD_ARG;
    static thread_local std::vector<uint64_t> r;
    r.resize((size_t)nslots);
    for (int i = 0; i < nslots; ++i) {
        const unsigned k = reloc[i];
        if (k == ALM_LIST_LITERAL) r[i] = slots[i];
        else if (k == ALM_LIST_STREAM) r[i] = (uint64_t)(uintptr_t)stream;
        else if (k == ALM_LIST_HOST_PTRS || k == ALM_LIST_HOST_INTS) r[i] = 0;
        else if ((int)k <= nbases) r[i] = bases[k - 1] + slots[i];
        else return ALM_ERR_BAD_ARG;
    }
    for (int i = 0; i < nslots; ++i) {
        const unsigned k = reloc[i];
        if (k != ALM_LIST_HOST_PTRS && k != ALM_LIST_HOST_INTS) continue;
        const uint64_t at = slots[i];
        if (at >= (uint64_t)nslots) return ALM_ERR_BAD_ARG;
        r[i] = (uint64_t)(uintptr_t)(k == ALM_LIST_HOST_PTRS ? (const void*)&r[at] : (const void*)&slots[at]);
    }
    for (int e = 0; e < n; ++e) {
        const AlmListEntry& en = entries[e];
        if (en.op < 0 || en.op >= NOPS || en.nargs != OPS[en.op].nargs || en.first < 0 || en.first + en.nargs > nslots) {
            if (failed_at) *failed_at = e;
            return ALM_ERR_BAD_ARG;
        }
        const int rc = OPS[en.op].thunk(r.data() + en.first);
        if (rc != 0) {
            if (failed_at) *failed_at = e;
            return rc;
        }
    }
    return 0;
}

}
```

audiolm-pytorch_amd/csrc/norm_act.hip:

```cpp
#include "common.hpp"
#include "../../include/audiolm_hip.h"

namespace {

constexpr float LN_EPS = 1e-5f;

__device__ __forceinline__ float4 load4(const float* p) { return *reinterpret_cast<const float4*>(p); }
__device__ __forceinline__ float4 load4(const bf16_t* p) {
    const uint2 u = *reinterpret_cast<const uint2*>(p);
    return make_float4(__uint_as_float(u.x << 16), __uint_as_float(u.x & 0xffff0000u), __uint_as_float(u.y << 16),
                       __uint_as_float(u.y & 0xffff0000u));
}
__device__ __forceinline__ void store4(float* p, float4 v) { *reinterpret_cast<float4*>(p) = v; }
__device__ __forceinline__ void store4(bf16_t* p, float4 v) {
    *reinterpret_cast<uint2*>(p) = make_uint2(pack_bf2(v.x, v.y), pack_bf2(v.z, v.w));
}

template <typename TIN, typename TOUT, int NI>
__global__ __launch_bounds__(256) void ln_fwd_kernel(const TIN* __restrict__ x, long long ldx, const float* __restrict__ gamma,
                                                     TOUT* __restrict__ y, long long ldy, bf16_t* __restrict__ xcopy, long long ldc,
                                                     float* __restrict__ mean_out, float* __restrict__ rstd_out, int rows, int D) {
    const int lane = threadIdx.x & 63;
    const int wpb = blockDim.x >> 6;
    for (int row = blockIdx.x * wpb + (threadIdx.x >> 6); row < rows; row += gridDim.x * wpb) {
        float4 v[NI];
        float s = 0.f;
#pragma unroll
        for (int i = 0; i < NI; ++i) {
            const int e = (i * 64 + lane) * 4;
            v[i] = (e < D) ? load4(x + (long long)row * ldx + e) : make_float4(0.f, 0.f, 0.f, 0.f);
            s += v[i].x + v[i].y + v[i].z + v[i].w;
        }
        const float mean = wave_sum(s) / (float)D;
        float q = 0.f;
#pragma unroll
        for (int i = 0; i < NI; ++i) {
            const int e = (i * 64 + lane) * 4;
            if (e < D) {
                const float a = v[i].x - mean, b = v[i].y - mean, c = v[i].z - mean, d = v[i].w - mean;
                q += a * a + b * b + c * c + d * d;
            }
        }
        const float rstd = rsqrtf(wave_sum(q) / (float)D + LN_EPS);
#pragma unroll
        for (int i = 0; i < NI; ++i) {
            const int e = (i * 64 + lane) * 4;
            if (e < D) {
                const float4 g = load4(gamma + e);
                store4(y + (long long)row * ldy + e,
                       make_float4((v[i].x - mean) * rstd * g.x, (v[i].y - mean) * rstd * g.y, (v[i].z - mean) * rstd * g.z,
                                   (v[i].w - mean) * rstd * g.w));
                if (xcopy) store4(xcopy + (long long)row * ldc + e, v[i]);
            }
        }
        if (lane == 0) {
            mean_out[row] = mean;
            rstd_out[row] = rstd;
        }
    }
}

template <typename TDY, typename TX, typename TDX, int NI>
__global__ __launch_bounds__(256) void ln_bwd_kernel(const TDY* __restrict__ dy, long long lddy, const TX* __restrict__ x, long long ldx,
                                                     const float* __restrict__ mean_in, const float* __restrict__ rstd_in,
                                                     const float* __restrict__ gamma, const bf16_t* __restrict__ extra, long long lde,
                                                     TDX* __restrict__ dx, long long lddx, float* __restrict__ dgamma_part, int rows, int D) {
    __shared__ float red[4][NI * 256];
    const int lane = threadIdx.x & 63, wave = threadIdx.x >> 6;
    float4 dg[NI];
#pragma unroll
    for (int i = 0; i < NI; ++i) dg[i] = make_float4(0.f, 0.f, 0.f, 0.f);
    for (int row = blockIdx.x * 4 + wave; row < rows; row += gridDim.x * 4) {
        const float mean = mean_in[row], rstd = rstd_in[row];
        float4 xh[NI], g[NI];
        float s1 = 0.f, s2 = 0.f;
#pragma unroll
        for (int i = 0; i < NI; ++i) {
            const int e = (i * 64 + lane) * 4;
            if (e < D) {
                const float4 xv = load4(x + (long long)row * ldx + e);
                const float4 d = load4(dy + (long long)row * lddy + e);
                const float4 gm = load4(gamma + e);
                xh[i] = make_float4((xv.x - mean) * rstd, (xv.y - mean) * rstd, (xv.z - mean) * rstd, (xv.w - mean) * rstd);
                g[i] = make_float4(d.x * gm.x, d.y * gm.y, d.z * gm.z, d.w * gm.w);
                dg[i].x += d.x * xh[i].x; dg[i].y += d.y * xh[i].y; dg[i].z += d.z * xh[i].z; dg[i].w += d.w * xh[i].w;
                s1 += g[i].x + g[i].y + g[i].z + g[i].w;
                s2 += g[i].x * xh[i].x + g[i].y * xh[i].y + g[i].z * xh[i].z + g[i].w * xh[i].w;
            } else {
                xh[i] = g[i] = make_float4(0.f, 0.f, 0.f, 0.f);
            }
        }
        const float c1 = wave_sum(s1) / (float)D, c2 = wave_sum(s2) / (float)D;
#pragma unroll
        for (int i = 0; i < NI; ++i) {
            const int e = (i * 64 + lane) * 4;
            if (e < D) {
                float4 o = make_float4(rstd * (g[i].x - c1 - xh[i].x * c2), rstd * (g[i].y - c1 - xh[i].y * c2),
                                       rstd * (g[i].z - c1 - xh[i].z * c2), rstd * (g[i].w - c1 - xh[i].w * c2));
                if (extra) {
                    const float4 ex = load4(extra + (long long)row * lde + e);
                    o.x += ex.x; o.y += ex.y; o.z += ex.z; o.w += ex.w;
                }
                store4(dx + (long long)row * lddx + e, o);
            }
        }
    }
    if (!dgamma_part) return;
#pragma unroll
    for (int i = 0; i < NI; ++i) *reinterpret_cast<float4*>(&red[wave][(i * 64 + lane) * 4]) = dg[i];
    __syncthreads();
    for (int e = threadIdx.x; e < D; e += 256)
        dgamma_part[(long long)blockIdx.x * D + e] = red[0][e] + red[1][e] + red[2][e] + red[3][e];
}

template <typename T>
__global__ __launch_bounds__(256) void colsum_kernel(const T* __restrict__ in, long long ld, int rows, int cols, float* __restrict__ out,
                                                     float scale, int accumulate, int rows_per_chunk, int direct) {
    __shared__ float red[4][64];
    const int cx = threadIdx.x & 63, ry = threadIdx.x >> 6;
    const int c = blockIdx.x * 64 + cx;
    const int r0 = blockIdx.y * rows_per_chunk, r1 = min(rows, r0 + rows_per_chunk);
    float s0 = 0.f, s1 = 0.f, s2 = 0.f, s3 = 0.f;
    auto ldv = [&](int r) -> float {
        if constexpr (sizeof(T) == 2) return bf2f(in[(long long)r * ld + c]);
        else return in[(long long)r * ld + c];
    };
    if (c < cols) {
        int r = r0 + ry;
        for (; r + 12 < r1; r += 16) {
            s0 += ldv(r); s1 += ldv(r + 4); s2 += ldv(r + 8); s3 += ldv(r + 12);
        }
        for (; r < r1; r += 4) s0 += ldv(r);
    }
    red[ry][cx] = (s0 + s1) + (s2 + s3);
    __syncthreads();
    if (ry == 0 && c < cols) {
        const float v = (red[0][cx] + red[1][cx]) + (red[2][cx] + red[3][cx]);
        if (direct) out[c] = accumulate ? out[c] + v * scale : v * scale;
        else out[(long long)blockIdx.y * cols + c] = v;
    }
}

__global__ __launch_bounds__(256) void colsum_finish_kernel(const float* __restrict__ ws, int chunks, int cols, float* __restrict__ out, float scale,
                                                            int accumulate) {
    const int c = blockIdx.x * 256 + threadIdx.x;
    if (c >= cols) return;
    float v = 0.f;
    for (int k = 0; k < chunks; ++k) v += ws[(long long)k * cols + c];
    v *= scale;
    out[c] = accumulate ? out[c] + v : v;
}

__device__ __forceinline__ float& f4e(float4& v, int c) { return reinterpret_cast<float*>(&v)[c]; }
__device__ __forceinline__ float f4e(const float4& v, int c) { return reinterpret_cast<const float*>(&v)[c]; }

constexpr int GE_MAX = 3;

__device__ __forceinline__ float block_sum256(float v, float* red) {
    v = wave_sum(v);
    if ((threadIdx.x & 63) == 0) red[threadIdx.x >> 6] = v;
    __syncthreads();
    return red[0] + red[1] + red[2] + red[3];
}
__device__ __forceinline__ void block_sum256x2(float& a, float& b, float* red) {
    a = wave_sum(a);
    b = wave_sum(b);
    if ((threadIdx.x & 63) == 0) { red[threadIdx.x >> 6] = a; red[4 + (threadIdx.x >> 6)] = b; }
    __syncthreads();
    a = red[0] + red[1] + red[2] + red[3];
    b = red[4] + red[5] + red[6] + red[7];
}

__global__ __launch_bounds__(256) void geglu_ln_fwd_kernel(const bf16_t* __restrict__ u, long long ldu, int goff, const float* __restrict__ gamma,
                                                           bf16_t* __restrict__ out, long long ldo, float* __restrict__ mean_out,
                                                           float* __restrict__ rstd_out, int rows, int I, int Ipad) {
    __shared__ float red[4][4];
    const int t = threadIdx.x;
    float4 gam[GE_MAX];
#pragma unroll
    for (int j = 0; j < GE_MAX; ++j) {
        const int e = (t + 256 * j) * 4;
        gam[j] = make_float4(e < I ? gamma[e] : 0.f, e + 1 < I ? gamma[e + 1] : 0.f, e + 2 < I ? gamma[e + 2] : 0.f, e + 3 < I ? gamma[e + 3] : 0.f);
    }
    struct Raw { uint2 x[GE_MAX], g[GE_MAX]; };
    auto issue = [&](Raw& r, int row) {
#pragma unroll
        for (int j = 0; j < GE_MAX; ++j) {
            const int e = (t + 256 * j) * 4;
            r.x[j] = r.g[j] = make_uint2(0u, 0u);
            if (e < Ipad && row < rows) {
                r.x[j] = *reinterpret_cast<const uint2*>(u + (long long)row * ldu + e);
                r.g[j] = *reinterpret_cast<const uint2*>(u + (long long)row * ldu + goff + e);
            }
        }
    };
    auto cvt = [](uint2 v) {
        return make_float4(__uint_as_float(v.x << 16), __uint_as_float(v.x & 0xffff0000u), __uint_as_float(v.y << 16), __uint_as_float(v.y & 0xffff0000u));
    };
    auto process = [&](const Raw& r, int row, int par) {
        float4 h[GE_MAX];
        float s = 0.f;
#pragma unroll
        for (int j = 0; j < GE_MAX; ++j) {
            const int e = (t + 256 * j) * 4;
            h[j] = make_float4(0.f, 0.f, 0.f, 0.f);
            if (e < Ipad) {
                const float4 xv = cvt(r.x[j]);
                const float4 gv = cvt(r.g[j]);
#pragma unroll
                for (int c = 0; c < 4; ++c) {
                    float cdf, pdf;
                    gauss_cdf_pdf(f4e(gv, c), cdf, pdf);
                    f4e(h[j], c) = (e + c < I) ? f4e(gv, c) * cdf * f4e(xv, c) : 0.f;
                }
                s += h[j].x + h[j].y + h[j].z + h[j].w;
            }
        }
        const float mean = block_sum256(s, red[par]) / (float)I;
        float q = 0.f;
#pragma unroll
        for (int j = 0; j < GE_MAX; ++j) {
            const int e = (t + 256 * j) * 4;
            if (e < I) {
                const float a = h[j].x - mean, b = h[j].y - mean, c = h[j].z - mean, d = h[j].w - mean;
                q += a * a + (e + 1 < I ? b * b : 0.f) + (e + 2 < I ? c * c : 0.f) + (e + 3 < I ? d * d : 0.f);
            }
        }
        const float rstd = rsqrtf(block_sum256(q, red[par + 1]) / (float)I + LN_EPS);
#pragma unroll
        for (int j = 0; j < GE_MAX; ++j) {
            const int e = (t + 256 * j) * 4;
            if (e < Ipad) {
                float4 o;
// ... 164 lines not shown
        const long long r = e / I;
        const int c = (int)(e % I);
        const float xv = x[r * 2 * I + c], g = x[r * 2 * I + I + c], d = dy[e];
        dx[r * 2 * I + c] = d * gelu_f(g);
        dx[r * 2 * I + I + c] = d * xv * gelu_grad_f(g);
    }
}

}

extern "C" int alm_ln_partial_blocks(int rows) { return min((rows + 3) / 4, 512); }

extern "C" int alm_layernorm_fwd(const void* x, int x_is_bf16, long long ldx, const float* gamma, void* y, int y_is_f32, long long ldy, void* xcopy,
                                 long long ldc, float* mean, float* rstd, int rows, int D, void* stream) {
    if (rows <= 0) return 0;
    if ((D & 3) || (ldx & 3) || (ldy & 3) || (xcopy && (ldc & 3))) return ALM_ERR_BAD_ARG;
    hipStream_t st = (hipStream_t)stream;
    int rc;
    if (y_is_f32)
        rc = x_is_bf16 ? launch_ln_fwd((const bf16_t*)x, ldx, gamma, (float*)y, ldy, (bf16_t*)xcopy, ldc, mean, rstd, rows, D, st)
                       : launch_ln_fwd((const float*)x, ldx, gamma, (float*)y, ldy, (bf16_t*)xcopy, ldc, mean, rstd, rows, D, st);
    else
        rc = x_is_bf16 ? launch_ln_fwd((const bf16_t*)x, ldx, gamma, (bf16_t*)y, ldy, (bf16_t*)xcopy, ldc, mean, rstd, rows, D, st)
                       : launch_ln_fwd((const float*)x, ldx, gamma, (bf16_t*)y, ldy, (bf16_t*)xcopy, ldc, mean, rstd, rows, D, st);
    if (rc) return rc;
    ALM_LAUNCH_CHECK();
    return 0;
}

extern "C" int alm_layernorm_bwd(const void* dy, int dy_is_f32, long long lddy, const void* x, int x_is_bf16, long long ldx, const float* mean,
                                 const float* rstd, const float* gamma, const void* extra, long long lde, void* dx, int dx_is_bf16,
                                 long long lddx, float* dgamma_part, int rows, int D, void* stream) {
    if (rows <= 0) return 0;
    if ((D & 3) || (ldx & 3) || (lddy & 3) || (lddx & 3) || (extra && (lde & 3))) return ALM_ERR_BAD_ARG;
    const int grid = alm_ln_partial_blocks(rows);
    hipStream_t st = (hipStream_t)stream;
    int rc;
    if (dy_is_f32) {
        if (x_is_bf16 || dx_is_bf16) return ALM_ERR_UNSUPPORTED;
        rc = launch_ln_bwd((const float*)dy, lddy, (const float*)x, ldx, mean, rstd, gamma, (const bf16_t*)extra, lde, (float*)dx, lddx, dgamma_part, grid, rows, D, st);
    } else if (x_is_bf16 && dx_is_bf16)
        rc = launch_ln_bwd((const bf16_t*)dy, lddy, (const bf16_t*)x, ldx, mean, rstd, gamma, (const bf16_t*)extra, lde, (bf16_t*)dx, lddx, dgamma_part, grid, rows, D, st);
    else if (x_is_bf16)
        rc = launch_ln_bwd((const bf16_t*)dy, lddy, (const bf16_t*)x, ldx, mean, rstd, gamma, (const bf16_t*)extra, lde, (float*)dx, lddx, dgamma_part, grid, rows, D, st);
    else if (dx_is_bf16)
        rc = launch_ln_bwd((const bf16_t*)dy, lddy, (const float*)x, ldx, mean, rstd, gamma, (const bf16_t*)extra, lde, (bf16_t*)dx, lddx, dgamma_part, grid, rows, D, st);
    else
        rc = launch_ln_bwd((const bf16_t*)dy, lddy, (const float*)x, ldx, mean, rstd, gamma, (const bf16_t*)extra, lde, (float*)dx, lddx, dgamma_part, grid, rows, D, st);
    if (rc) return rc;
    ALM_LAUNCH_CHECK();
    return 0;
}

extern "C" int alm_colsum_chunks(int rows);
extern "C" int alm_colsum_partial(const float* in, long long ld, int rows, int cols, float* ws, void* stream) {
    if (cols <= 0 || rows <= 0 || !ws) return ALM_ERR_BAD_ARG;
    const int chunks = alm_colsum_chunks(rows);
    const int rpc = (rows + chunks - 1) / chunks;
    hipLaunchKernelGGL(colsum_kernel<float>, dim3((cols + 63) / 64, chunks), dim3(256), 0, (hipStream_t)stream, in, ld, rows, cols, ws, 1.f, 0, rpc, 0);
    ALM_LAUNCH_CHECK();
    return 0;
}

extern "C" int alm_colsum_chunks(int rows) { return rows <= 128 ? 1 : min(16, (rows + 63) / 64); }

extern "C" int alm_colsum(const void* in, int in_is_bf16, long long ld, int rows, int cols, float* out, float scale, int accumulate, float* ws,
                          void* stream) {
    if (cols <= 0) return 0;
    const int chunks = ws ? alm_colsum_chunks(rows) : 1;
    const int rpc = (rows + chunks - 1) / chunks;
    const int direct = chunks == 1;
    dim3 grid((cols + 63) / 64, chunks);
    float* o1 = direct ? out : ws;
    if (in_is_bf16)
        hipLaunchKernelGGL(colsum_kernel<bf16_t>, grid, dim3(256), 0, (hipStream_t)stream, (const bf16_t*)in, ld, rows, cols, o1, scale, accumulate, rpc, direct);
    else
        hipLaunchKernelGGL(colsum_kernel<float>, grid, dim3(256), 0, (hipStream_t)stream, (const float*)in, ld, rows, cols, o1, scale, accumulate, rpc, direct);
    if (!direct)
        hipLaunchKernelGGL(colsum_finish_kernel, dim3((cols + 255) / 256), dim3(256), 0, (hipStream_t)stream, ws, chunks, cols, out, scale, accumulate);
    ALM_LAUNCH_CHECK();
    return 0;
}

extern "C" int alm_geglu_partial_blocks(int rows) { return min(rows, 1024); }

extern "C" int alm_geglu_ln_fwd(const void* u, long long ldu, int gate_offset, const float* gamma, void* out, long long ldo, float* mean,
                                float* rstd, int rows, int inner, int inner_pad, void* stream) {
    if (rows <= 0) return 0;
    if (inner <= 0 || inner_pad < inner || inner_pad > GE_MAX * 1024 || (inner_pad & 7) || (ldu & 7) || (gate_offset & 7)) return ALM_ERR_UNSUPPORTED;
    hipLaunchKernelGGL(geglu_ln_fwd_kernel, dim3(min(rows, 2048)), dim3(256), 0, (hipStream_t)stream, (const bf16_t*)u, ldu, gate_offset, gamma,
                       (bf16_t*)out, ldo, mean, rstd, rows, inner, inner_pad);
    ALM_LAUNCH_CHECK();
    return 0;
}

extern "C" int alm_geglu_ln_bwd(const void* dhn, long long lddh, const void* u, long long ldu, int gate_offset, const float* gamma,
                                const float* mean, const float* rstd, void* du, float* dgamma_part, int rows, int inner, int inner_pad,
                                void* stream) {
    if (rows <= 0) return 0;
    if (inner <= 0 || inner_pad < inner || inner_pad > GE_MAX * 1024 || (inner_pad & 7) || (ldu & 7) || (gate_offset & 7)) return ALM_ERR_UNSUPPORTED;
    hipLaunchKernelGGL(geglu_ln_bwd_kernel, dim3(alm_geglu_partial_blocks(rows)), dim3(256), 0, (hipStream_t)stream, (const bf16_t*)dhn, lddh,
                       (const bf16_t*)u, ldu, gate_offset, gamma, mean, rstd, (bf16_t*)du, dgamma_part, rows, inner, inner_pad);
    ALM_LAUNCH_CHECK();
    return 0;
}

extern "C" int alm_geglu_fwd(const float* x, float* y, long long rows, int inner, void* stream) {
    if (rows <= 0 || inner <= 0) return 0;
    const long long n = rows * inner;
    hipLaunchKernelGGL(geglu_fwd_kernel, dim3((unsigned)min((n + 255) / 256, (long long)8192)), dim3(256), 0, (hipStream_t)stream, x, y, rows, inner);
    ALM_LAUNCH_CHECK();
    return 0;
}

extern "C" int alm_geglu_bwd(const float* dy, const float* x, float* dx, long long rows, int inner, void* stream) {
    if (rows <= 0 || inner <= 0) return 0;
    const long long n = rows * inner;
    hipLaunchKernelGGL(geglu_bwd_kernel, dim3((unsigned)min((n + 255) / 256, (long long)8192)), dim3(256), 0, (hipStream_t)stream, dy, x, dx, rows, inner);
    ALM_LAUNCH_CHECK();
    return 0;
}
```

audiolm-pytorch_amd/launchlist.py:

```python
from __future__ import annotations

import bisect
import ctypes
import dataclasses
import math
import os
import struct
import sys

import torch

from . import _lib, ops

ENABLED = os.environ.get('ALM_LAUNCH_LIST', '1') != '0'
MAX_ARENA_BYTES = int(float(os.environ.get('ALM_LAUNCH_LIST_MAX_GB', '24')) * (1 << 30))
MAX_PLANS = max(1, int(os.environ.get('ALM_LAUNCH_LIST_MAX_PLANS', '64')))
ALIGN = 256
LITERAL, STREAM, HOST_PTRS, HOST_INTS = 0, 0xFFFF, 0xFFFE, 0xFFFD
_P, _I, _L, _F, _U = _lib._P, _lib._I, _lib._L, _lib._F, _lib._U
_M64 = (1 << 64) - 1

STATS = dict(sized=0, recorded=0, replayed=0, refused=0)


# ... 145 lines not shown
                elif isinstance(a, ctypes.Array):
                    arrays.append((len(self.slots), a))
                    self.slots.append(0), self.reloc.append(LITERAL)
                elif isinstance(a, int):
                    bid, off = self._classify(a, f'{name} argument {i}')
                    self.slots.append(off), self.reloc.append(bid)
                else:
                    self.fail(f'{name} argument {i}: {type(a).__name__} is not a device pointer')
                    self.slots.append(0), self.reloc.append(LITERAL)
            elif t is _F:
                self.slots.append(struct.unpack('<I', struct.pack('<f', float(a)))[0]), self.reloc.append(LITERAL)
            else:
                self.slots.append(int(a) & _M64), self.reloc.append(LITERAL)
        for at, arr in arrays:
            here = len(self.slots)
            if arr._type_ is ctypes.c_void_p:
                for j, v in enumerate(arr):
                    if v is None:
                        self.slots.append(0), self.reloc.append(LITERAL)
                    else:
                        bid, off = self._classify(int(v), f'{name} host array element {j}')
                        self.slots.append(off), self.reloc.append(bid)
                self.slots[at], self.reloc[at] = here, HOST_PTRS
            elif arr._type_ is ctypes.c_int:
                vals = [int(v) & 0xFFFFFFFF for v in arr] + [0]
                for j in range(0, len(vals) - 1, 2):
                    self.slots.append(vals[j] | (vals[j + 1] << 32)), self.reloc.append(LITERAL)
                self.slots[at], self.reloc[at] = here, HOST_INTS
            else:
                self.fail(f'{name}: host array of {arr._type_.__name__}')
        self.entries.append((op, len(sig), first))
        self.names.append(name)

    def finish(self, arena_bytes):
        rec = Recorded(self.entries, self.slots, self.reloc, self.nbases, arena_bytes)
        rec.names = self.names
        return rec


def _spec(t, arena, rec):
    if t is None:
        return None
    off = t.data_ptr() - arena.base
    if not (0 <= off and off + _extent(t) <= arena.cap) or off % t.element_size():
        rec.fail('an output of the pass does not live in its arena')
        return None
    return (off // t.element_size(), t.dtype, tuple(t.shape), tuple(t.stride()))


def _rebuild(spec, typed):
    if spec is None:
        return None
    off, dtype, shape, stride = spec
    return typed[dtype].as_strided(shape, stride, off)


def _typed(buf):
    return {torch.float32: buf.view(torch.float32), torch.bfloat16: buf.view(torch.bfloat16)}



class Plan:
    def __init__(self, key):
        self.key = key
        self.state = 'size'
        self.fwd_bytes = self.bwd_bytes = None
        self.fwd = self.bwd = None
        self.why = None
        self.dhn_dtype = None
        self.orphans = 0


class Replay:

    def __init__(self, plan, arena, xin):
        self.plan, self.arena, self.xin = plan, arena, xin


PLANS = {}


def _switches(core):
    return (core.QKV_GROUP, core.QKV_GROUP_MAX_M, core.ASYNC_KV, core.DEFER_WGRAD, core.DEFER_GROUPS, core.DEFER_GROUP_SIZES, core.DEFER_MAX_BYTES, core.HC_BATCH_FINISH,
            core.PACK_ALL, core.ASYNC_WGRAD, core.SIDE_STREAMS, ops.NT_WS)


def plan_for(core, x, mask_u8, cfg, need, bias, nflat, defer, dx_scale):
    if not ENABLED:
        return None
    dev = x.device
    key = (dev.index, ops._st(), tuple(x.shape), need, mask_u8 is None, None if bias is None else int(bias.tbl.shape[1]), dataclasses.astuple(cfg), nflat,
           bool(defer), float(dx_scale), _switches(core))
    plan = PLANS.pop(key, None)
    if plan is None:
        plan = Plan(key)
        while len(PLANS) >= MAX_PLANS:
            PLANS.pop(next(iter(PLANS)))
    PLANS[key] = plan
    return None if plan.state == 'off' else plan


def _weight_images(core, cache, cfg):
    out = []
    for l in range(cfg.depth):
        for kind in core.branch_kinds(cfg):
            for name in ('wq', 'wkv', 'wo', 'w1', 'w2'):
                hit = cache.store.get((l, kind, name))
                if hit is not None:
                    out += [hit[1][0], hit[1][1]]
    return out


def _bias_tensors(bias):
    return [] if bias is None else [bias.tbl, bias.qkey4, bias.kkey4, bias.qattr, bias.kattr]


def _turn_off(plan, why):
    plan.state, plan.why, plan.fwd, plan.bwd = 'off', why, None, None
    STATS['refused'] += 1
    print(f'[audiolm_pytorch_amd] launch list refused for a stack shape (the eager path stays in use): {why}', file=sys.stderr, flush=True)


def _fill(rec, first, tensors):
    b = rec.bases
    for i, t in enumerate(tensors, first):
        b[i] = 0 if t is None else t.data_ptr()


def forward(core, plan, xin, mask_u8, flat, cfg, cache, need, bias, defer):
    kw = dict(defer_wgrad=defer)
    if plan.state == 'ready' and (plan.bwd is not None or not need):
        core.pack_stack_weights(cache, flat, cfg)
        rec = plan.fwd
        arena = torch.empty(rec.arena_bytes, dtype=torch.uint8, device=xin.device)
        rec.bases[0] = arena.data_ptr()
        _fill(rec, 1, [xin, mask_u8] + _bias_tensors(bias) + list(flat) + _weight_images(core, cache, cfg))
        rec.run(ops._st())
        STATS['replayed'] += 1
        hn = _rebuild(rec.outputs, _typed(arena))
        return hn, (Replay(plan, arena, xin) if need else None)
    core.pack_stack_weights(cache, flat, cfg)
    if plan.state == 'size':
        tally = _Tally()
        ops.ALLOC = tally
        try:
            hn, saved = core.stack_forward(xin, mask_u8, flat, cfg, cache, need, bias, **kw)
        finally:
            ops.ALLOC = None
        plan.fwd_bytes = tally.bytes
        STATS['sized'] += 1
        if tally.bytes > MAX_ARENA_BYTES:
            _turn_off(plan, f'forward arena of {tally.bytes / 2 ** 30:.1f} GB exceeds ALM_LAUNCH_LIST_MAX_GB')
        elif not need:
            plan.state = 'record'
        if saved is not None:
            saved['_ll'] = (plan, 'size', None, xin)
        return hn, saved
    plan.orphans += 1
    if plan.orphans > 8:
        _turn_off(plan, 'forwards with gradients enabled whose backward never ran')
        return core.stack_forward(xin, mask_u8, flat, cfg, cache, need, bias, **kw)
    bases = [None, xin, mask_u8] + _bias_tensors(bias) + list(flat) + _weight_images(core, cache, cfg)
    arena = _Arena(plan.fwd_bytes, xin.device)
    bases[0] = (arena.base, arena.cap)
    rec = Recorder(bases, ops._st())
    arena.recorder = rec
    ops.ALLOC, _lib.RECORDER = arena, rec
# ... 73 lines not shown
```

audiolm-pytorch_amd/ops.py:

```python
from __future__ import annotations

import ctypes
import os

import torch

from . import _lib

BF16, F32 = torch.bfloat16, torch.float32


_raw_stream = getattr(torch._C, '_cuda_getCurrentRawStream', None)
_cur_dev = getattr(torch._C, '_cuda_getDevice', None) or torch.cuda.current_device


def _st():
    if _raw_stream is not None:
        return _raw_stream(_cur_dev())
    return torch.cuda.current_stream().cuda_stream


def _chk(t, dtype=None):
    if not t.is_cuda:
        raise _lib.AlmError('audiolm_pytorch_amd ops run on the MI355X only (got a CPU tensor); there is no CPU fallback')
    if dtype is not None and t.dtype != dtype:
        raise _lib.AlmError(f'expected {dtype}, got {t.dtype}')
    if t.device.index != _cur_dev():
        raise _lib.AlmError(f'tensor on cuda:{t.device.index} but the current device is cuda:{torch.cuda.current_device()}: call '
                            'torch.cuda.set_device(...) (one process per GPU) before using audiolm_pytorch_amd')
    return t


def _p(t):
    return None if t is None else t.data_ptr()


ALLOC = None


def _new(shape, dtype=None, device=None):
    if ALLOC is not None:
        return ALLOC.empty(shape, dtype, device)
    return torch.empty(shape, dtype=dtype, device=device)


def _new_zeros(shape, dtype=None, device=None):
    if ALLOC is not None:
        return ALLOC.zeros(shape, dtype, device)
    return torch.zeros(shape, dtype=dtype, device=device)


def _new_like(t):
    if ALLOC is not None and t.is_contiguous():
        return ALLOC.empty(t.shape, t.dtype, t.device)
    return torch.empty_like(t)


def memset_zero(t):
    assert t.is_contiguous()
    _lib.call('alm_memset_zero', t.data_ptr(), t.numel() * t.element_size(), _st())
    return t


def persistent_buffers():
    return list(_NT_WS.values())


def _rows_ld(t):
    assert t.dim() == 2 and t.stride(1) == 1, (t.shape, t.stride())
    return t.shape[0], t.shape[1], t.stride(0)



_NT_WS = {}
NT_WS = os.environ.get('ALM_GEMM_NT_WS', '1') != '0'


def _nt_ws(dev, stream):
    key = (dev.index, stream)
    ws = _NT_WS.get(key)
    if ws is None:
        ws = _NT_WS[key] = torch.zeros(_lib.query('alm_gemm_nt_ws_bytes'), dtype=torch.uint8, device=dev)
    return ws


def gemm_nt(A, B, C, *, bias=None, alpha=1.0, accumulate=False):
    _chk(A, BF16), _chk(B, BF16), _chk(C)
    assert A.stride(-1) == 1 and B.stride(-1) == 1 and C.stride(-1) == 1
    nb = A.dim() - 2
    assert nb in (0, 1, 2) and B.dim() == A.dim() and C.dim() == A.dim()
    M, K = A.shape[-2:]
    N = B.shape[-2]
    assert B.shape[-1] == K and C.shape[-2] == M and C.shape[-1] == N, (A.shape, B.shape, C.shape)
    bs = [1, 1]
    sa, sb, sc = [0, 0], [0, 0], [0, 0]
    for i in range(nb):
        j = 2 - nb + i
        bs[j] = A.shape[i]
        sa[j], sb[j], sc[j] = A.stride(i), B.stride(i) if B.shape[i] != 1 else 0, C.stride(i)
    st = _st()
    if NT_WS and M >= 256 and N >= 256:
        ws = _nt_ws(A.device, st)
        _lib.call('alm_gemm_bf16_nt_ws', A.data_ptr(), B.data_ptr(), C.data_ptr(), _p(bias), M, N, K, A.stride(-2), B.stride(-2), C.stride(-2),
                  bs[0], bs[1], sa[0], sa[1], sb[0], sb[1], sc[0], sc[1], float(alpha), int(C.dtype == F32), int(accumulate), ws.data_ptr(), ws.numel(), st)
    else:
        _lib.call('alm_gemm_bf16_nt', A.data_ptr(), B.data_ptr(), C.data_ptr(), _p(bias), M, N, K, A.stride(-2), B.stride(-2), C.stride(-2),
                  bs[0], bs[1], sa[0], sa[1], sb[0], sb[1], sc[0], sc[1], float(alpha), int(C.dtype == F32), int(accumulate), st)
    return C


def gemm_nt_inl(A, B, C, slices, *, bias=None, alpha=1.0, accumulate=False):
    _chk(A, BF16), _chk(B, BF16), _chk(C)
    M, K = A.shape
    N = B.shape[0]
    st = _st()
    ws = _nt_ws(A.device, st)
    _lib.call('alm_gemm_bf16_nt_inl', A.data_ptr(), B.data_ptr(), C.data_ptr(), _p(bias), M, N, K, A.stride(0), B.stride(0), C.stride(0),
              float(alpha), int(C.dtype == F32), int(accumulate), int(slices), ws.data_ptr(), ws.numel(), st)
    return C


def gemm_nt_group2(A0, B0, C0, A1, B1, C1):
    for t in (A0, B0, A1, B1):
        _chk(t, BF16)
        assert t.dim() == 2 and t.stride(1) == 1
    _chk(C0), _chk(C1)
    assert C0.dtype == C1.dtype and C0.stride(1) == 1 and C1.stride(1) == 1
    (M0, K0), (M1, K1), N0, N1 = A0.shape, A1.shape, B0.shape[0], B1.shape[0]
    assert B0.shape[1] == K0 and B1.shape[1] == K1 and tuple(C0.shape) == (M0, N0) and tuple(C1.shape) == (M1, N1)
    _lib.call('alm_gemm_bf16_nt_group2', A0.data_ptr(), B0.data_ptr(), C0.data_ptr(), M0, N0, K0, A0.stride(0), B0.stride(0), C0.stride(0),
              A1.data_ptr(), B1.data_ptr(), C1.data_ptr(), M1, N1, K1, A1.stride(0), B1.stride(0), C1.stride(0), int(C0.dtype == F32), _st())
    return C0, C1


def _splitk(name, A, B, C, M, N, K, nb, sA, sB, sC, alpha, accumulate):
    nws = _lib.query('alm_gemm_splitk_ws_floats', M, N, K, nb)
    if nws < 0:
        raise _lib.AlmError('split-K workspace exceeds 2^31 floats')
    ws = _new(nws, dtype=F32, device=A.device) if nws > 0 else None
    _lib.call(name, A.data_ptr(), B.data_ptr(), C.data_ptr(), _p(ws), M, N, K, A.stride(-2), B.stride(-2), C.stride(-2), nb, sA, sB, sC,
              float(alpha), int(accumulate), _st())
    return C


def gemm_nt_splitk(A, B, C, *, alpha=1.0, accumulate=False):
    _chk(A, BF16), _chk(B, BF16), _chk(C, F32)
    M, K = A.shape
    N = B.shape[0]
    assert B.shape[1] == K and C.shape == (M, N) and A.stride(1) == 1 and B.stride(1) == 1 and C.stride(1) == 1
    return _splitk('alm_gemm_bf16_nt_splitk', A, B, C, M, N, K, 1, 0, 0, 0, alpha, accumulate)


def gemm_tn_splitk(At, Bt, C, *, alpha=1.0, accumulate=False):
    _chk(At, BF16), _chk(Bt, BF16), _chk(C, F32)
    nb, sA, sC = 1, 0, 0
    if At.dim() == 3:
        nb, sA, sC = At.shape[0], At.stride(0), C.stride(0)
        assert C.dim() == 3 and C.shape[0] == nb
    K, M = At.shape[-2:]
    N = Bt.shape[1]
    assert Bt.dim() == 2 and Bt.shape[0] == K and C.shape[-2:] == (M, N) and At.stride(-1) == 1 and Bt.stride(1) == 1 and C.stride(-1) == 1
    return _splitk('alm_gemm_bf16_tn_splitk', At, Bt, C, M, N, K, nb, sA, 0, sC, alpha, accumulate)


def gemm_tn_batched(At, Bt, C, *, alpha=1.0, accumulate=False):
    _chk(At, BF16), _chk(Bt, BF16), _chk(C, F32)
    assert At.dim() == 4 and Bt.dim() == 4 and C.dim() == 4 and At.stride(-1) == 1 and Bt.stride(-1) == 1 and C.stride(-1) == 1
    n1, n2, K, M = At.shape
    N = Bt.shape[-1]
    assert Bt.shape[-2] == K and tuple(C.shape) == (n1, n2, M, N), (At.shape, Bt.shape, C.shape)
    sb = [Bt.stride(0) if Bt.shape[0] != 1 else 0, Bt.stride(1) if Bt.shape[1] != 1 else 0]
    nws = _lib.query('alm_gemm_splitk_ws_floats', M, N, K, n1 * n2)
    if nws < 0:
        raise _lib.AlmError('split-K workspace exceeds 2^31 floats')
    ws = _new(nws, dtype=F32, device=At.device) if nws > 0 else None
    _lib.call('alm_gemm_bf16_tn_batched', At.data_ptr(), Bt.data_ptr(), C.data_ptr(), _p(ws), M, N, K, At.stride(-2), Bt.stride(-2), C.stride(-2), n1, n2,
              At.stride(0), At.stride(1), sb[0], sb[1], C.stride(0), C.stride(1), float(alpha), int(accumulate), _st())
    return C


def gemm_nt_tile(A, B, C, tile, *, bias=None, alpha=1.0, accumulate=False):
    _chk(A, BF16), _chk(B, BF16), _chk(C)
    M, K = A.shape
    N = B.shape[0]
    _lib.call('alm_gemm_bf16_nt_tile', A.data_ptr(), B.data_ptr(), C.data_ptr(), _p(bias), M, N, K, A.stride(0), B.stride(0), C.stride(0),
              float(alpha), int(C.dtype == F32), int(accumulate), int(tile), _st())
    return C


def transpose(src, rows_pad=None):
    _chk(src, BF16)
    rows, cols, ld = _rows_ld(src)
    rp = rows_pad or ((rows + 7) // 8 * 8)
    dst = _new((cols, rp), dtype=BF16, device=src.device)
    _lib.call('alm_transpose_bf16', src.data_ptr(), dst.data_ptr(), rows, cols, ld, rp, rp, _st())
    return dst


def pack_weight(w, dst=None, dstT=None, rows_pad=None, cols_pad=None):
    _chk(w, F32)
    rows, cols, ld = _rows_ld(w)
    rp, cp = rows_pad or rows, cols_pad or cols
    _lib.call('alm_pack_weight', w.data_ptr(), rows, cols, ld, _p(dst), dst.stride(0) if dst is not None else 0, rp, cp,
              _p(dstT), dstT.stride(0) if dstT is not None else 0, _st())


def pack_weights_multi(jobs):
    arr = (_lib.AlmPackJob * len(jobs))()
    for i, (w, dst, dstT, rp, cp) in enumerate(jobs):
        _chk(w, F32)
        rows, cols, ld = _rows_ld(w)
        arr[i] = _lib.AlmPackJob(w.data_ptr(), rows, cols, ld, _p(dst), dst.stride(0) if dst is not None else 0, rp, cp,
                                 _p(dstT), dstT.stride(0) if dstT is not None else 0)
    _lib.call('alm_pack_weights_multi', ctypes.cast(arr, ctypes.c_void_p), len(jobs), _st())



def layernorm_fwd(x, gamma, *, want_copy=False, out_f32=False, y_out=None, xc_out=None):
    _chk(x)
    rows, D, ld = _rows_ld(x)
    y = _new((rows, D), dtype=F32 if out_f32 else BF16, device=x.device) if y_out is None else y_out
    xc = (_new((rows, D), dtype=BF16, device=x.device) if xc_out is None else xc_out) if want_copy else None
    assert y.shape == (rows, D) and y.is_contiguous() and (xc is None or (xc.shape == (rows, D) and xc.is_contiguous()))
    mean = _new(rows, dtype=F32, device=x.device)
    rstd = _new(rows, dtype=F32, device=x.device)
    _lib.call('alm_layernorm_fwd', x.data_ptr(), int(x.dtype == BF16), ld, gamma.data_ptr(), y.data_ptr(), int(out_f32), D, _p(xc), D, mean.data_ptr(),
              rstd.data_ptr(), rows, D, _st())
    return y, xc, mean, rstd


def colsum(inp, out=None, scale=1.0, accumulate=False):
    _chk(inp)
    rows, cols, ld = _rows_ld(inp)
    if out is None:
        out = _new(cols, dtype=F32, device=inp.device)
    chunks = _lib.query('alm_colsum_chunks', rows)
    ws = _new((chunks, cols), dtype=F32, device=inp.device) if chunks > 1 else None
    _lib.call('alm_colsum', inp.data_ptr(), int(inp.dtype == BF16), ld, rows, cols, out.data_ptr(), float(scale), int(accumulate), _p(ws), _st())
    return out


def layernorm_bwd(dy, x, mean, rstd, gamma, *, extra=None, dx_dtype=F32, want_dgamma=True):
    _chk(dy), _chk(x)
    assert dy.dtype in (BF16, F32)
    rows, D, lddy = _rows_ld(dy)
    dx = _new((rows, D), dtype=dx_dtype, device=dy.device)
    part = None
    if want_dgamma:
        nblk = _lib.query('alm_ln_partial_blocks', rows)
        part = _new((nblk, D), dtype=F32, device=dy.device)
    _lib.call('alm_layernorm_bwd', dy.data_ptr(), int(dy.dtype == F32), lddy, x.data_ptr(), int(x.dtype == BF16), x.stride(0), mean.data_ptr(), rstd.data_ptr(),
              gamma.data_ptr(), _p(extra), extra.stride(0) if extra is not None else 0, dx.data_ptr(), int(dx_dtype == BF16), D, _p(part),
              rows, D, _st())
    return dx, (colsum(part) if want_dgamma else None)


def geglu_fwd(x):
    _chk(x, F32)
    rows, two_i, ld = _rows_ld(x)
    assert ld == two_i and two_i % 2 == 0
    y = _new((rows, two_i // 2), dtype=F32, device=x.device)
    _lib.call('alm_geglu_fwd', x.data_ptr(), y.data_ptr(), rows, two_i // 2, _st())
    return y


def geglu_bwd(dy, x):
    _chk(dy, F32), _chk(x, F32)
    rows, two_i, ld = _rows_ld(x)
    assert ld == two_i and dy.shape == (rows, two_i // 2) and dy.is_contiguous()
    dx = _new_like(x)
    _lib.call('alm_geglu_bwd', dy.data_ptr(), x.data_ptr(), dx.data_ptr(), rows, two_i // 2, _st())
    return dx


def geglu_ln_fwd(u, gamma, inner, inner_pad, out=None):
    _chk(u, BF16)
    rows, _, ldu = _rows_ld(u)
    if out is None:
        out = _new((rows, inner_pad), dtype=BF16, device=u.device)
    assert out.shape == (rows, inner_pad) and out.dtype == BF16 and out.stride(1) == 1 and out.stride(0) == inner_pad
    mean = _new(rows, dtype=F32, device=u.device)
    rstd = _new(rows, dtype=F32, device=u.device)
    _lib.call('alm_geglu_ln_fwd', u.data_ptr(), ldu, inner_pad, gamma.data_ptr(), out.data_ptr(), inner_pad, mean.data_ptr(), rstd.data_ptr(),
              rows, inner, inner_pad, _st())
    return out, mean, rstd


def geglu_ln_bwd(dhn, u, gamma, mean, rstd, inner, inner_pad, du_out=None):
    rows, _, ldu = _rows_ld(u)
    du = _new_like(u) if du_out is None else du_out
    assert du.shape == u.shape and du.stride(0) == ldu and du.stride(1) == 1 and du.dtype == BF16
    nblk = _lib.query('alm_geglu_partial_blocks', rows)
    part = _new((nblk, inner), dtype=F32, device=u.device)
    _lib.call('alm_geglu_ln_bwd', dhn.data_ptr(), dhn.stride(0), u.data_ptr(), ldu, inner_pad, gamma.data_ptr(), mean.data_ptr(), rstd.data_ptr(),
              du.data_ptr(), part.data_ptr(), rows, inner, inner_pad, _st())
    return du, colsum(part)



def _bias_args(bias, N, H):
    tbl = _chk(bias.tbl, F32)
    assert tbl.dim() == 2 and tbl.shape[0] == H and tbl.is_contiguous(), tbl.shape
    for t in (bias.qkey4, bias.kkey4, bias.qattr, bias.kattr):
        _chk(t, torch.int32)
        assert t.shape == (N,) and t.is_contiguous(), (t.shape, N)
    return (tbl.data_ptr(), tbl.shape[1], bias.qkey4.data_ptr(), bias.kkey4.data_ptr(), bias.qattr.data_ptr(), bias.kattr.data_ptr())


def attn_bias_part(B, N, H, LT, device):
    return _new_zeros((_lib.query('alm_attn_bias_part_rows', B, N, H), LT), dtype=F32, device=device)


def attn_bias_grad_reduce(part, B, N, H, dim_head=64):
    LT = part.shape[1]
    dtbl = _new((H, LT), dtype=F32, device=part.device)
    _lib.call('alm_attn_bias_grad_reduce', part.data_ptr(), dtbl.data_ptr(), B, N, H, LT, float(dim_head) ** -0.5, _st())
    return dtbl


def mqa_attn_fwd(q, k, v, mask, B, N, H, dim_head=64, bias=None, dropout_p=0., seed=0, o=None, seed_dev=None):
    _chk(q, BF16), _chk(k, BF16), _chk(v, BF16)
    if o is None:
        o = _new((B * N, H * dim_head), dtype=BF16, device=q.device)
    assert o.shape == (B * N, H * dim_head) and o.dtype == BF16 and o.stride(1) == 1
    lse = _new((B, H, N), dtype=F32, device=q.device)
    if bias is not None:
        _lib.call('alm_mqa_attn_bias_fwd', q.data_ptr(), q.stride(0), k.data_ptr(), k.stride(0), v.data_ptr(), v.stride(0), _p(mask), o.data_ptr(),
                  o.stride(0), lse.data_ptr(), B, N, H, dim_head, float(dim_head) ** -0.5, *_bias_args(bias, N, H), float(dropout_p), int(seed), _p(seed_dev), _st())
        return o, lse
    _lib.call('alm_mqa_attn_fwd', q.data_ptr(), q.stride(0), k.data_ptr(), k.stride(0), v.data_ptr(), v.stride(0), _p(mask), o.data_ptr(),
              o.stride(0), lse.data_ptr(), B, N, H, dim_head, float(dim_head) ** -0.5, float(dropout_p), int(seed), _p(seed_dev), _st())
    return o, lse


def mqa_attn_bwd(q, k, v, mask, o, lse, dout, B, N, H, dim_head=64, bias=None, dtbl_part=None, dropout_p=0., seed=0, dq_out=None, seed_dev=None):
    _chk(dout, BF16)
    dq = _new_like(q) if dq_out is None else dq_out
    assert dq.shape == q.shape and dq.dtype == BF16 and dq.stride(1) == 1
    hg = _lib.query('alm_mqa_bwd_parts', B, N, H)
    dkv = _new((hg, B * N, 2 * dim_head), dtype=F32, device=q.device)
    delta = _new((2, B, H, N), dtype=F32, device=q.device)
    if bias is not None:
        assert dtbl_part is not None and dtbl_part.shape[1] == bias.tbl.shape[1] and dtbl_part.is_contiguous()
        _lib.call('alm_mqa_attn_bias_bwd', q.data_ptr(), q.stride(0), k.data_ptr(), k.stride(0), v.data_ptr(), v.stride(0), _p(mask),
                  o.data_ptr(), o.stride(0), lse.data_ptr(), dout.data_ptr(), dout.stride(0), dq.data_ptr(), dq.stride(0), dkv.data_ptr(),
                  dkv.data_ptr() + 4 * dim_head, dkv.stride(1), dkv.stride(0), delta.data_ptr(), B, N, H, dim_head, float(dim_head) ** -0.5,
                  *_bias_args(bias, N, H), dtbl_part.data_ptr(), float(dropout_p), int(seed), _p(seed_dev), _st())
        return dq, dkv
    _lib.call('alm_mqa_attn_bwd', q.data_ptr(), q.stride(0), k.data_ptr(), k.stride(0), v.data_ptr(), v.stride(0), _p(mask), o.data_ptr(),
              o.stride(0), lse.data_ptr(), dout.data_ptr(), dout.stride(0), dq.data_ptr(), dq.stride(0), dkv.data_ptr(),
              dkv.data_ptr() + 4 * dim_head, dkv.stride(1), dkv.stride(0), delta.data_ptr(), B, N, H, dim_head, float(dim_head) ** -0.5,
              float(dropout_p), int(seed), _p(seed_dev), _st())
    return dq, dkv


def mqa_decode_attn(q, cache, kv_new, pos, mask, H, dim_head=64, bias=None, pos_dev=None):
    _chk(q, BF16), _chk(cache, BF16), _chk(kv_new, BF16)
    B, Nmax = cache.shape[0], cache.shape[1]
    assert cache.is_contiguous() and cache.shape[2] == 2 * dim_head and kv_new.shape == (B, 2 * dim_head) and kv_new.stride(1) == 1
    out = _new((B, H * dim_head), dtype=BF16, device=q.device)
    qk = qa = 0
    tb = (None, 0)
    vecs = (None, None, None, None)
    if bias is not None:
        tbl = _chk(bias.tbl, F32)
        assert tbl.is_contiguous() and tbl.shape[0] == H and bias.kkey4.shape[0] >= Nmax
        tb = (tbl.data_ptr(), tbl.shape[1])
        if pos_dev is None:
            qk, qa = int(bias.qkey4_host[pos]), int(bias.qattr_host[pos])
        vecs = (bias.kkey4.data_ptr(), bias.kattr.data_ptr(), bias.qkey4.data_ptr(), bias.qattr.data_ptr())
    _lib.call('alm_mqa_decode_attn', q.data_ptr(), q.stride(0), cache.data_ptr(), cache.stride(0), kv_new.data_ptr(), kv_new.stride(0), _p(mask),
              mask.stride(0) if mask is not None else 0, out.data_ptr(), out.stride(0), B, H, dim_head, int(pos), Nmax, float(dim_head) ** -0.5,
              tb[0], tb[1], qk, qa, vecs[0], vecs[1], _p(pos_dev), vecs[2] if pos_dev is not None else None,
              vecs[3] if pos_dev is not None else None, _st())
    return out


def value_residual_mix(v, v0):
# ... 816 lines not shown
```

include/audiolm_hip.h:

```cpp
#pragma once
#ifdef __cplusplus
extern "C" {
#endif

#define ALM_ERR_BAD_ARG 10001
#define ALM_ERR_UNSUPPORTED 10002

int alm_gemm_bf16_nt(const void* A, const void* B, void* C, const float* bias, int M, int N, int K, long long lda, long long ldb,
                     long long ldc, int nb1, int nb2, long long sA1, long long sA2, long long sB1, long long sB2, long long sC1,
                     long long sC2, float alpha, int out_f32, int accumulate, void* stream);
int alm_gemm_bf16_nt_ws(const void* A, const void* B, void* C, const float* bias, int M, int N, int K, long long lda, long long ldb, long long ldc,
                        int nb1, int nb2, long long sA1, long long sA2, long long sB1, long long sB2, long long sC1, long long sC2, float alpha,
                        int out_f32, int accumulate, void* ws, long long ws_bytes, void* stream);
int alm_gemm_bf16_nt_inl(const void* A, const void* B, void* C, const float* bias, int M, int N, int K, long long lda, long long ldb, long long ldc,
                         float alpha, int out_f32, int accumulate, int slices, void* ws, long long ws_bytes, void* stream);
int alm_gemm_nt_plan(int M, int N, int K, int nb, int with_ws, int* plan);
int alm_gemm_nt_ws_bytes(void);
int alm_gemm_bf16_nt_group2(const void* A0, const void* B0, void* C0, int M0, int N0, int K0, long long lda0, long long ldb0, long long ldc0,
                            const void* A1, const void* B1, void* C1, int M1, int N1, int K1, long long lda1, long long ldb1, long long ldc1,
                            int out_f32, void* stream);
int alm_gemm_bf16_nt_tile(const void* A, const void* B, void* C, const float* bias, int M, int N, int K, long long lda, long long ldb,
                          long long ldc, float alpha, int out_f32, int accumulate, int tile, void* stream);
int alm_gemm_splitk_slices(int M, int N, int K, int nb);
int alm_gemm_splitk_ws_floats(int M, int N, int K, int nb);
int alm_gemm_splitk_tile(int M, int N, int K, int nb);
int alm_gemm_nt_tile_choice(int M, int N, int nb);
int alm_gemm_tn_batched_plan(int M, int N, int K, int nb, int* plan);
int alm_gemm_bf16_nt_splitk(const void* A, const void* B, float* C, float* ws, int M, int N, int K, long long lda, long long ldb,
                            long long ldc, int nb, long long sA, long long sB, long long sC, float alpha, int accumulate, void* stream);
int alm_gemm_bf16_tn_splitk(const void* At, const void* Bt, float* C, float* ws, int M, int N, int K, long long lda, long long ldb,
                            long long ldc, int nb, long long sA, long long sB, long long sC, float alpha, int accumulate, void* stream);
int alm_gemm_bf16_tn_batched(const void* At, const void* Bt, float* C, float* ws, int M, int N, int K, long long lda, long long ldb, long long ldc,
                             int nb1, int nb2, long long sA1, long long sA2, long long sB1, long long sB2, long long sC1, long long sC2, float alpha,
                             int accumulate, void* stream);
int alm_transpose_bf16(const void* src, void* dst, int rows, int cols, long long ld_src, long long ld_dst, int rows_pad, void* stream);
int alm_transpose_bf16_batched(const void* src, void* dst, int rows, int cols, long long ld_src, long long ld_dst, int rows_pad, int nb,
                               long long bs_src, long long bs_dst, void* stream);
int alm_pack_weight(const float* src, int rows, int cols, long long ld_src, void* dst, long long ld_dst, int rows_pad, int cols_pad,
                    void* dstT, long long ld_dstT, void* stream);

typedef struct {
    const float* src; int rows, cols; long long ld_src;
    void* dst; long long ld_dst; int rows_pad, cols_pad;
    void* dstT; long long ld_dstT;
} AlmPackJob;
int alm_pack_weights_multi(const AlmPackJob* jobs, int njobs, void* stream);

int alm_ln_partial_blocks(int rows);
int alm_layernorm_fwd(const void* x, int x_is_bf16, long long ldx, const float* gamma, void* y, int y_is_f32, long long ldy, void* xcopy_bf16,
                      long long ldc, float* mean, float* rstd, int rows, int D, void* stream);
int alm_layernorm_bwd(const void* dy, int dy_is_f32, long long lddy, const void* x, int x_is_bf16, long long ldx, const float* mean,
                      const float* rstd, const float* gamma, const void* extra_bf16, long long lde, void* dx, int dx_is_bf16,
                      long long lddx, float* dgamma_part, int rows, int D, void* stream);
int alm_colsum(const void* in, int in_is_bf16, long long ld, int rows, int cols, float* out, float scale, int accumulate, float* ws,
               void* stream);
int alm_colsum_chunks(int rows);
int alm_colsum_partial(const float* in, long long ld, int rows, int cols, float* ws, void* stream);

int alm_geglu_fwd(const float* x, float* y, long long rows, int inner, void* stream);
int alm_geglu_bwd(const float* dy, const float* x, float* dx, long long rows, int inner, void* stream);
int alm_geglu_partial_blocks(int rows);
int alm_geglu_ln_fwd(const void* u_bf16, long long ldu, int gate_offset, const float* gamma, void* out_bf16, long long ldo, float* mean,
                     float* rstd, int rows, int inner, int inner_pad, void* stream);
int alm_geglu_ln_bwd(const void* dhn_bf16, long long lddh, const void* u_bf16, long long ldu, int gate_offset, const float* gamma,
                     const float* mean, const float* rstd, void* du_bf16, float* dgamma_part, int rows, int inner, int inner_pad,
                     void* stream);

int alm_mqa_attn_fwd(const void* q, long long ldq, const void* k, long long ldk, const void* v, long long ldv, const unsigned char* mask,
                     void* o, long long ldo, float* lse, int B, int N, int H, int dim_head, float scale, float dropout_p,
                     unsigned long long seed, const void* seed_dev, void* stream);
int alm_mqa_attn_bwd(const void* q, long long ldq, const void* k, long long ldk, const void* v, long long ldv, const unsigned char* mask,
                     const void* o, long long ldo, const float* lse, const void* dout, long long lddo, void* dq, long long lddq, float* dk,
                     float* dv, long long lddk, long long part_stride, float* delta, int B, int N, int H, int dim_head, float scale,
                     float dropout_p, unsigned long long seed, const void* seed_dev, void* stream);
int alm_mqa_head_groups(int H);
int alm_mqa_bwd_parts(int B, int N, int H);
int alm_mqa_attn_bias_fwd(const void* q, long long ldq, const void* k, long long ldk, const void* v, long long ldv, const unsigned char* mask,
                          void* o, long long ldo, float* lse, int B, int N, int H, int dim_head, float scale, const float* tbl, int LT,
                          const int* qkey4, const int* kkey4, const int* qattr, const int* kattr, float dropout_p, unsigned long long seed,
                          const void* seed_dev, void* stream);
int alm_mqa_attn_bias_bwd(const void* q, long long ldq, const void* k, long long ldk, const void* v, long long ldv, const unsigned char* mask,
                          const void* o, long long ldo, const float* lse, const void* dout, long long lddo, void* dq, long long lddq,
                          float* dk, float* dv, long long lddk, long long part_stride, float* delta, int B, int N, int H, int dim_head,
                          float scale, const float* tbl, int LT, const int* qkey4, const int* kkey4, const int* qattr, const int* kattr,
                          float* dtbl_part, float dropout_p, unsigned long long seed, const void* seed_dev, void* stream);
int alm_attn_bias_part_rows(int B, int N, int H);
int alm_attn_bias_grad_reduce(const float* dtbl_part, float* dtbl, int B, int N, int H, int LT, float scale, void* stream);
int alm_posmlp_in_fwd(const float* x, const float* W, const float* b, float* pre, void* act_bf16, int L, int in_dim, int C, void* stream);
int alm_posmlp_in_bwd_chunks(int L);
int alm_posmlp_in_bwd(const void* dpre_bf16, const float* x, float* partial, int L, int in_dim, int C, void* stream);
int alm_silu_fwd(const float* pre, void* act_bf16, long long n, void* stream);
int alm_silu_bwd(const float* dact, const float* pre, void* dpre_bf16, long long n, void* stream);
int alm_posmlp_out_fwd(const void* act_bf16, const float* W, const float* b, const float* special, float* tbl, int L, int C, int H,
                       float inv_scale, void* stream);
int alm_posmlp_out_bwd(const float* dtbl, const float* W, const float* pre, void* g_bf16, void* dpre_bf16, float* dspecial, int L, int C, int H,
                       int Hp, float inv_scale, void* stream);
int alm_xattn_softmax_fwd(const float* S, long long ldS, const unsigned char* emask, const float* lse_self, float scale, void* P_bf16, long long ldP,
                          float* lse_tot, float* fself, const float* bias, long long ldbias, int causal_off, int B, int N, int H, int Me, void* stream);
int alm_xattn_dbias(const void* P_bf16, long long ldP, const float* dP, long long lddP, const float* ndelta, float* dbias, long long lddb, int Me, int B,
                    int N, int H, void* stream);
int alm_xattn_combine(const void* o_self_bf16, long long ldos, const float* fself, const float* o_e, void* out_bf16, long long ldo, long long tokens,
                      int H, int dim_head, void* stream);
int alm_xattn_softmax_bwd(const void* P_bf16, long long ldP, const float* dP, long long lddP, const float* ndelta, float scale, void* dS_bf16,
                          long long lddS, int Me, int B, int N, int H, void* stream);
int alm_xattn_delta(const void* o_bf16, long long ldo, const void* dout_bf16, long long lddo, float* ndelta, int B, int N, int H, int dim_head,
                    void* stream);
int alm_value_residual_mix(const void* v, long long ldv, const void* v0, long long ldv0, void* out, long long ldo, long long rows,
                           int dim_head, void* stream);
int alm_kv_grad_pack(const float* dk, const float* dv, long long ld, int nparts, long long part_stride, float* acc_v0, void* dkv_bf16,
                     long long ldo, long long rows, int dim_head, int mode, void* stream);

int alm_loss_combine(const float* s0, const float* s1, const float* s2, const float* s3, const long long* l0, const long long* l1, const long long* l2,
                     const long long* l3, long long n0, long long n1, long long n2, long long n3, float w0, float w1, float w2, float w3, int G,
                     long long ignore_index, float* loss, float* scales, void* stream);

int alm_coarse_prepare(const long long* sem, long long ld_sem, const long long* coarse, long long ld_coarse, int B, int ns0, int nc0, long long pad_id,
                       long long sem_eos, long long coarse_eos, int Q, int C, long long* sem_labels, long long* coarse_labels, int* src_a, void* keep,
                       int sem_has_eos, void* stream);
int alm_semantic_prepare(const long long* sem, long long ld_sem, int B, int n0, long long eos_id, long long num_rows, long long* labels, int* src_a,
                         int has_eos, void* stream);
int alm_unique_consecutive_i64(const long long* ids, long long ld, int B, int n, int append_eos, long long eos_id, long long pad, long long* out,
                               long long ld_out, int* lengths, void* stream);
int alm_fine_prepare(const long long* coarse, long long ld_coarse, const long long* fine, long long ld_fine, int B, int n, int nf, long long pad_id,
                     long long eos_id, int Qc, int Qf, int C, int* src_a, void* keep, void* stream);

int alm_forgetful_mask(const float* score, long long ld_score, void* keep, long long ld_keep, int B, int N, int drop, void* stream);

int alm_hc_coef_width(int S);
int alm_hc_partial_width(int S, int D);
int alm_hc_grads_width(int S, int D);
int alm_hc_partial_rows(int mode, int fused_ln, int r_bf16, int S, long long tokens, int D);
int alm_hc_fwd(const void* R_in, int rin_bcast, int r_bf16, const void* y_prev_bf16, long long ldy, const float* coef_prev, void* R_out,
               const float* hc_gamma, const float* Wa, const float* sa, const float* Aa, const float* wb, const float* sb, const float* Bb,
               const float* ln_gamma, void* x_out_bf16, long long ldx, void* xn_out_bf16, long long ldxn, float* xn32_out, float* mean,
               float* rstd, float* coef, float* xs_out, int mode, int B, int S, int N, int D, void* stream);
int alm_hc_bwd(const void* dRn, int dRn_bcast, int r_bf16, const float* dx, long long lddx, const void* dxn_bf16, long long lddxn,
               const void* extra_bf16, long long ldex, const float* mean, const float* rstd, const float* ln_gamma, const void* R, int r_bcast,
               const float* coef, const float* dbeta, const float* hc_gamma, const float* Wa, const float* sa, const float* wb, const float* sb,
               void* dR, float* dsum, float dsum_scale, float* partial, const void* y_prev_bf16, long long ldy, const float* coef_prev, void* dy_bf16, long long lddy,
               float* dbeta_out, int mode, int B, int S, int N, int D, void* stream);
// ... 116 lines not shown
```

Measured before the change: 1.462 million audio-tokens/s.

## Batch deferred colsum and split-K reduce finishes into one multi-job kernel pair

Adds a FinishList that collects the LayerNorm and GEGLU-LN dgamma column-sum reductions, plus the split-K slab reductions of the batched weight-gradient GEMMs. It runs all of them at the end of the backward pass as one table-driven stage1/stage2 kernel launch instead of many small per-op reduce kernels. The goal is fewer tiny kernel launches and better GPU fill inside the captured graph. The cost is that split-K workspaces and partial buffers stay alive until the end of the backward pass, and the gradients are only finished at that point.

After: 1.461 million audio-tokens/s. No clear change (-0.1%).

```diff
diff --git a/audiolm-pytorch_amd/_lib.py b/audiolm-pytorch_amd/_lib.py
--- a/audiolm-pytorch_amd/_lib.py
+++ b/audiolm-pytorch_amd/_lib.py
@@ -23,6 +23,8 @@
     'alm_gemm_bf16_nt_splitk': [_P, _P, _P, _P, _I, _I, _I, _L, _L, _L, _I, _L, _L, _L, _F, _I, _P],
     'alm_gemm_bf16_tn_splitk': [_P, _P, _P, _P, _I, _I, _I, _L, _L, _L, _I, _L, _L, _L, _F, _I, _P],
     'alm_gemm_bf16_tn_batched': [_P, _P, _P, _P, _I, _I, _I, _L, _L, _L, _I, _I, _L, _L, _L, _L, _L, _L, _F, _I, _P],
+    'alm_gemm_bf16_tn_batched_partial': [_P, _P, _P, _P, _I, _I, _I, _L, _L, _L, _I, _I, _L, _L, _L, _L, _L, _L, _F, _I, _P],
+    'alm_gemm_tn_batched_reduce': [_I, _I, _I, _I, _I, _L, _L, _L, _P],
     'alm_gemm_bf16_nt_group2': [_P, _P, _P, _I, _I, _I, _L, _L, _L, _P, _P, _P, _I, _I, _I, _L, _L, _L, _I, _P],
     'alm_gemm_bf16_nt_tile': [_P, _P, _P, _P, _I, _I, _I, _L, _L, _L, _F, _I, _I, _I, _P],
     'alm_transpose_bf16': [_P, _P, _I, _I, _L, _L, _I, _P],
@@ -35,6 +37,8 @@
     'alm_colsum': [_P, _I, _L, _I, _I, _P, _F, _I, _P, _P],
     'alm_colsum_chunks': [_I],
     'alm_colsum_partial': [_P, _L, _I, _I, _P, _P],
+    'alm_finish_batched_ws_floats': [_P, _I],
+    'alm_finish_batched': [_P, _P, _P, _I, _P, _L, _P],
     'alm_geglu_fwd': [_P, _P, _L, _I, _P],
     'alm_geglu_bwd': [_P, _P, _P, _L, _I, _P],
     'alm_geglu_partial_blocks': [_I],
diff --git a/audiolm-pytorch_amd/core.py b/audiolm-pytorch_amd/core.py
--- a/audiolm-pytorch_amd/core.py
+++ b/audiolm-pytorch_amd/core.py
@@ -581,7 +581,7 @@
     return 0 if acc is None else (1 if mixed else 2)
 
 
-def ff_backward(cfg, W, prm, sv, dY, side, want_trace=False, du_out=None):
+def ff_backward(cfg, W, prm, sv, dY, side, want_trace=False, du_out=None, finish=None):
     M, D = dY.shape
     I, Ip, dev = cfg.inner, cfg.inner_pad, dY.device
     (_, W1T), (_, W2T) = W['w1'], W['w2']
@@ -597,7 +597,7 @@
         dW2 = _empty((D, I), F32, dev)
         HNs, dYs = sv['HN'], dY
         run(lambda: ops.gemm_tn_splitk(dYs, HNs[:, :I], dW2, alpha=fa), dYs, HNs, dW2)
-    dU, dg3 = ops.geglu_ln_bwd(dHN, sv['U'], prm['ln3'], sv['mean3'], sv['rstd3'], I, Ip, du_out=du_out)
+    dU, dg3 = ops.geglu_ln_bwd(dHN, sv['U'], prm['ln3'], sv['mean3'], sv['rstd3'], I, Ip, du_out=du_out, finish=finish)
     dXN = _empty((M, D), BF16, dev)
     ops.gemm_nt(dU, W1T, dXN)
     dW1 = None
@@ -622,7 +622,9 @@
     brs = saved['branches']
     scale = float(dh) ** -0.5
 
-    dxs, dgam = ops.layernorm_bwd(dhn, saved['xs'], saved['fmean'], saved['frstd'], flat[-1])
+    stk = saved.get('stk')
+    fin = ops.FinishList(slabs=ops.FINISH_BATCHED >= 2) if (ops.FINISH_BATCHED and stk is not None and on_layer_grads is None) else None
+    dxs, dgam = ops.layernorm_bwd(dhn, saved['xs'], saved['fmean'], saved['frstd'], flat[-1], finish=fin)
     grads[-1] = dgam
     multi = cfg.add_value_residual and cfg.depth > 1
     acc_v0 = ops._new_zeros((M, dh), dtype=F32, device=dev) if multi else None
@@ -634,7 +636,6 @@
     ddense = torch.zeros_like(bias.tbl) if dense else None
     dR, bcast = dxs, S > 1
     dY = dbeta = None
-    stk = saved.get('stk')
     bst = None
     if stk is not None:
         L = cfg.depth
@@ -694,7 +695,7 @@
                 if ngroups > 1 or on_layer_grads is not None:
                     side.run(lambda At=At, Bt=Bt, C=C: ops.gemm_tn_batched(At, Bt, C), At, Bt, C)
                 else:
-                    ops.gemm_tn_batched(At, Bt, C)
+                    ops.gemm_tn_batched(At, Bt, C, finish=fin)
             for k in kinds:
                 for l in range(l0, l1):
                     g_ = wgg[k][l - l0]
@@ -751,7 +752,7 @@
         extra = None
         W = LW[kind]
         if kind == 'ff':
-            dXN, dW1, dg3, dW2, dHN, dU = ff_backward(cfg, W, prm, sv, dY, side, want_trace=True, du_out=bst['dU'][l] if bst is not None else None)
+            dXN, dW1, dg3, dW2, dHN, dU = ff_backward(cfg, W, prm, sv, dY, side, want_trace=True, du_out=bst['dU'][l] if bst is not None else None, finish=fin)
             grads[ip + 1], grads[ip + 2], grads[ip + 3] = dW1, dg3, dW2
             rec = dict(dY=dY, dHN=dHN, dU=dU, dXN=dXN, dW1=dW1, dg3=dg3, dW2=dW2) if TRACE is not None else None
         elif kind == 'cross':
@@ -877,6 +878,8 @@
             side.run_after_all(lambda: on_layer_grads(l, grads[base:base + ppl]), *[g for g in grads[base:base + ppl] if g is not None])
 
     finish_hc()
+    if fin is not None:
+        fin.run()
     dx = dR.view(B, N, D)
     dtbl = ddense if dense else (ops.attn_bias_grad_reduce(dtbl_part, B, N, H) if bias is not None else None)
     side.join()
diff --git a/audiolm-pytorch_amd/csrc/gemm.hip b/audiolm-pytorch_amd/csrc/gemm.hip
--- a/audiolm-pytorch_amd/csrc/gemm.hip
+++ b/audiolm-pytorch_amd/csrc/gemm.hip
@@ -3,6 +3,7 @@
 #include <type_traits>
 
 #include "common.hpp"
+#include "reduce.hpp"
 #include "../../include/audiolm_hip.h"
 
 #ifndef ALM_GEMM_AUX_A
@@ -953,29 +954,7 @@
                                                             int nb2 = 0x40000000, long long sC1 = 0) {
     ws += (long long)blockIdx.y * mn;
     C += (long long)(blockIdx.y / nb2) * sC1 + (long long)(blockIdx.y % nb2) * sC;
-    const bool vec = (N & 3) == 0 && (ldc & 3) == 0 && ((uintptr_t)C & 15) == 0 && (mn & 3) == 0 && (slice_stride & 3) == 0;
-    if (vec) {
-        const long long mn4 = mn >> 2;
-        for (long long i = (long long)blockIdx.x * 256 + threadIdx.x; i < mn4; i += (long long)gridDim.x * 256) {
-            float4 s = make_float4(0.f, 0.f, 0.f, 0.f);
-            for (int z = 0; z < splits; ++z) {
-                const float4 v = *reinterpret_cast<const float4*>(ws + (long long)z * slice_stride + i * 4);
-                s.x += v.x; s.y += v.y; s.z += v.z; s.w += v.w;
-            }
-            const long long e = i * 4, m = e / N, n = e % N;
-            float4* c = reinterpret_cast<float4*>(C + m * ldc + n);
-            if (accumulate) { const float4 w = *c; s.x += w.x; s.y += w.y; s.z += w.z; s.w += w.w; }
-            *c = s;
-        }
-        return;
-    }
-    for (long long i = (long long)blockIdx.x * 256 + threadIdx.x; i < mn; i += (long long)gridDim.x * 256) {
-        float s = 0.f;
-        for (int z = 0; z < splits; ++z) s += ws[(long long)z * slice_stride + i];
-        const long long m = i / N, n = i % N;
-        float* c = C + m * ldc + n;
-        *c = accumulate ? *c + s : s;
-    }
+    slab_reduce(ws, splits, mn, slice_stride, N, C, ldc, 1.f, accumulate, blockIdx.x, gridDim.x);
 }
 
 __global__ __launch_bounds__(256) void transpose_bf16_kernel(const bf16_t* __restrict__ src, bf16_t* __restrict__ dst, int rows, int cols,
@@ -1411,7 +1390,7 @@
 }
 
 int splitk_fixed(const bf16_t* At, const bf16_t* Bt, float* C, float* ws, int M, int N, int K, long long lda, long long ldb, long long ldc, int slices,
-                 float alpha, int accumulate, hipStream_t st) {
+                 float alpha, int accumulate, hipStream_t st, bool reduce = true) {
     int kc = (K + slices - 1) / slices;
     kc = (kc + BK - 1) / BK * BK;
     const int nsl = (K + kc - 1) / kc;
@@ -1419,9 +1398,16 @@
     GemmParams p{At, Bt, ws, nullptr, M, N, K, lda, ldb, (long long)N, 1, 0, 0, 0, 0, 0, mn, alpha, 0, kc, mn, 0, nsl, 1};
     int rc = launch_gemm<true>(p, 1, nsl, 1, 13, st);
     if (rc) return rc;
+    if (!reduce) return 0;
     const int grid = (int)((mn + 255) / 256 < 2048 ? (mn + 255) / 256 : 2048);
     hipLaunchKernelGGL(splitk_reduce_kernel, dim3(grid, 1), dim3(256), 0, st, (const float*)ws, nsl, mn, mn, N, C, ldc, 0LL, accumulate);
     return 0;
+}
+
+int splitk_nsl(int K, int slices) {
+    int kc = (K + slices - 1) / slices;
+    kc = (kc + BK - 1) / BK * BK;
+    return (K + kc - 1) / kc;
 }
 
 }
@@ -1624,9 +1610,9 @@
     return 0;
 }
 
-extern "C" int alm_gemm_bf16_tn_batched(const void* At, const void* Bt, float* C, float* ws, int M, int N, int K, long long lda, long long ldb,
-                                        long long ldc, int nb1, int nb2, long long sA1, long long sA2, long long sB1, long long sB2, long long sC1,
-                                        long long sC2, float alpha, int accumulate, void* stream) {
+static int tn_batched(const void* At, const void* Bt, float* C, float* ws, int M, int N, int K, long long lda, long long ldb,
+                      long long ldc, int nb1, int nb2, long long sA1, long long sA2, long long sB1, long long sB2, long long sC1,
+                      long long sC2, float alpha, int accumulate, void* stream, bool reduce) {
     if (M <= 0 || N <= 0 || nb1 <= 0 || nb2 <= 0) return 0;
     if (K <= 0 || (lda & 7) || (ldb & 7) || ((sA1 | sA2 | sB1 | sB2) & 7) || ((uintptr_t)At & 15) || ((uintptr_t)Bt & 15)) return ALM_ERR_BAD_ARG;
     if (view_too_big(K, lda) || view_too_big(K, ldb)) return ALM_ERR_UNSUPPORTED;
@@ -1648,7 +1634,7 @@
         float* C2 = C + zC + (hy.m_major ? (long long)hy.off * ldc : hy.off);
         const int M2 = hy.m_major ? M - hy.off : M, N2 = hy.m_major ? N : N - hy.off;
         if (!ws) return ALM_ERR_BAD_ARG;
-        rc = splitk_fixed(A2, B2, C2, ws, M2, N2, K, lda, ldb, ldc, hy.slices_b, alpha, accumulate, st);
+        rc = splitk_fixed(A2, B2, C2, ws, M2, N2, K, lda, ldb, ldc, hy.slices_b, alpha, accumulate, st, reduce);
         if (rc) return rc;
         ALM_LAUNCH_CHECK();
         return 0;
@@ -1668,11 +1654,41 @@
         rc = launch_gemm<true>(p, nb, nsl, 1, pl.tile, st);
         if (rc) return rc;
         const int grid = (int)((mn + 255) / 256 < 2048 ? (mn + 255) / 256 : 2048);
-        hipLaunchKernelGGL(splitk_reduce_kernel, dim3(grid, nb), dim3(256), 0, st, (const float*)ws, nsl, mn, mn * nb, N, C, ldc, sC2, accumulate, nb2, sC1);
+        if (reduce)
+            hipLaunchKernelGGL(splitk_reduce_kernel, dim3(grid, nb), dim3(256), 0, st, (const float*)ws, nsl, mn, mn * nb, N, C, ldc, sC2, accumulate, nb2, sC1);
     }
     if (rc) return rc;
     ALM_LAUNCH_CHECK();
     return 0;
+}
+
+extern "C" int alm_gemm_bf16_tn_batched(const void* At, const void* Bt, float* C, float* ws, int M, int N, int K, long long lda, long long ldb,
+                                        long long ldc, int nb1, int nb2, long long sA1, long long sA2, long long sB1, long long sB2, long long sC1,
+                                        long long sC2, float alpha, int accumulate, void* stream) {
+    return tn_batched(At, Bt, C, ws, M, N, K, lda, ldb, ldc, nb1, nb2, sA1, sA2, sB1, sB2, sC1, sC2, alpha, accumulate, stream, true);
+}
+
+extern "C" int alm_gemm_bf16_tn_batched_partial(const void* At, const void* Bt, float* C, float* ws, int M, int N, int K, long long lda, long long ldb,
+                                                long long ldc, int nb1, int nb2, long long sA1, long long sA2, long long sB1, long long sB2, long long sC1,
+                                                long long sC2, float alpha, int accumulate, void* stream) {
+    return tn_batched(At, Bt, C, ws, M, N, K, lda, ldb, ldc, nb1, nb2, sA1, sA2, sB1, sB2, sC1, sC2, alpha, accumulate, stream, false);
+}
+
+extern "C" int alm_gemm_tn_batched_reduce(int M, int N, int K, int nb1, int nb2, long long ldc, long long sC1, long long sC2, long long* r) {
+    if (M <= 0 || N <= 0 || K <= 0 || nb1 <= 0 || nb2 <= 0 || !r) return 0;
+    const int nb = nb1 * nb2;
+    const HybridPlan hy = hybrid_plan(M, N, K, nb);
+    if (hy.panels_a > 0) {
+        const long long M2 = hy.m_major ? M - hy.off : M, N2 = hy.m_major ? N : N - hy.off;
+        r[0] = (long long)(nb1 - 1) * sC1 + (long long)(nb2 - 1) * sC2 + (hy.m_major ? (long long)hy.off * ldc : hy.off);
+        r[1] = splitk_nsl(K, hy.slices_b); r[2] = N2; r[3] = ldc; r[4] = M2 * N2; r[5] = M2 * N2; r[6] = 1; r[7] = 0x40000000; r[8] = 0; r[9] = 0;
+        return 1;
+    }
+    const SplitPlan pl = splitk_plan(M, N, K, nb);
+    if (pl.slices <= 1) return 0;
+    const long long mn = (long long)M * N;
+    r[0] = 0; r[1] = splitk_nsl(K, pl.slices); r[2] = N; r[3] = ldc; r[4] = mn; r[5] = mn * nb; r[6] = nb; r[7] = nb2; r[8] = sC1; r[9] = sC2;
+    return 1;
 }
 
 extern "C" int alm_transpose_bf16(const void* src, void* dst, int rows, int cols, long long ld_src, long long ld_dst, int rows_pad,
diff --git a/audiolm-pytorch_amd/csrc/launchlist.hip b/audiolm-pytorch_amd/csrc/launchlist.hip
--- a/audiolm-pytorch_amd/csrc/launchlist.hip
+++ b/audiolm-pytorch_amd/csrc/launchlist.hip
@@ -56,10 +56,12 @@
     ALM_OP(alm_gemm_bf16_nt_splitk),
     ALM_OP(alm_gemm_bf16_tn_splitk),
     ALM_OP(alm_gemm_bf16_tn_batched),
+    ALM_OP(alm_gemm_bf16_tn_batched_partial),
     ALM_OP(alm_layernorm_fwd),
     ALM_OP(alm_layernorm_bwd),
     ALM_OP(alm_colsum),
     ALM_OP(alm_colsum_partial),
+    ALM_OP(alm_finish_batched),
     ALM_OP(alm_geglu_ln_fwd),
     ALM_OP(alm_geglu_ln_bwd),
     ALM_OP(alm_mqa_attn_fwd),
diff --git a/audiolm-pytorch_amd/csrc/norm_act.hip b/audiolm-pytorch_amd/csrc/norm_act.hip
--- a/audiolm-pytorch_amd/csrc/norm_act.hip
+++ b/audiolm-pytorch_amd/csrc/norm_act.hip
@@ -1,4 +1,7 @@
+#include <string.h>
+
 #include "common.hpp"
+#include "reduce.hpp"
 #include "../../include/audiolm_hip.h"
 
 namespace {
@@ -117,38 +120,58 @@
 __global__ __launch_bounds__(256) void colsum_kernel(const T* __restrict__ in, long long ld, int rows, int cols, float* __restrict__ out,
                                                      float scale, int accumulate, int rows_per_chunk, int direct) {
     __shared__ float red[4][64];
-    const int cx = threadIdx.x & 63, ry = threadIdx.x >> 6;
-    const int c = blockIdx.x * 64 + cx;
-    const int r0 = blockIdx.y * rows_per_chunk, r1 = min(rows, r0 + rows_per_chunk);
-    float s0 = 0.f, s1 = 0.f, s2 = 0.f, s3 = 0.f;
-    auto ldv = [&](int r) -> float {
-        if constexpr (sizeof(T) == 2) return bf2f(in[(long long)r * ld + c]);
-        else return in[(long long)r * ld + c];
-    };
-    if (c < cols) {
-        int r = r0 + ry;
-        for (; r + 12 < r1; r += 16) {
-            s0 += ldv(r); s1 += ldv(r + 4); s2 += ldv(r + 8); s3 += ldv(r + 12);
-        }
-        for (; r < r1; r += 4) s0 += ldv(r);
-    }
-    red[ry][cx] = (s0 + s1) + (s2 + s3);
-    __syncthreads();
-    if (ry == 0 && c < cols) {
-        const float v = (red[0][cx] + red[1][cx]) + (red[2][cx] + red[3][cx]);
-        if (direct) out[c] = accumulate ? out[c] + v * scale : v * scale;
-        else out[(long long)blockIdx.y * cols + c] = v;
-    }
+    colsum_stage1<T>(in, ld, rows, cols, out, scale, accumulate, rows_per_chunk, direct, blockIdx.x, blockIdx.y, red);
 }
 
 __global__ __launch_bounds__(256) void colsum_finish_kernel(const float* __restrict__ ws, int chunks, int cols, float* __restrict__ out, float scale,
                                                             int accumulate) {
-    const int c = blockIdx.x * 256 + threadIdx.x;
-    if (c >= cols) return;
-    float v = 0.f;
-    for (int k = 0; k < chunks; ++k) v += ws[(long long)k * cols + c];
-    v *= scale;
-    out[c] = accumulate ? out[c] + v : v;
+    colsum_stage2(ws, chunks, cols, out, scale, accumulate, blockIdx.x);
+}
+
+constexpr int FIN_MAX = 32;
+constexpr int FIN_COLSUM_F32 = 0, FIN_COLSUM_BF16 = 1, FIN_SLAB = 2;
+struct FinJob {
+    const void* in;
+    float* out;
+    float* ws;
+    int kind, a, b, ld;
+    int accumulate;
+    float scale;
+    int chunks;
+    int mn, slice_stride, nb, nb2, sC1, sC;
+};
+struct FinTable {
+    FinJob job[FIN_MAX];
+    int blk[FIN_MAX + 1];
+    int n;
+};
+__device__ __forceinline__ int fin_find_job(const FinTable& t) {
+    int j = 0;
+    while (j + 1 < t.n && (int)blockIdx.x >= t.blk[j + 1]) ++j;
+    return j;
+}
+__global__ __launch_bounds__(256) void finish_stage1_kernel(FinTable t) {
+    __shared__ float red[4][64];
+    const int j = fin_find_job(t);
+    const FinJob& q = t.job[j];
+    const int b = (int)blockIdx.x - t.blk[j];
+    if (q.kind == FIN_SLAB) {
+        const int y = b / q.chunks, x = b % q.chunks;
+        const float* ws = (const float*)q.in + (long long)y * q.mn;
+        float* C = q.out + (long long)(y / q.nb2) * q.sC1 + (long long)(y % q.nb2) * q.sC;
+        slab_reduce(ws, q.a, q.mn, q.slice_stride, q.b, C, q.ld, q.scale, q.accumulate, x, q.chunks);
+        return;
+    }
+    const int nbx = (q.b + 63) / 64, direct = q.chunks == 1;
+    const int rpc = (q.a + q.chunks - 1) / q.chunks;
+    float* o1 = direct ? q.out : q.ws;
+    if (q.kind == FIN_COLSUM_BF16) colsum_stage1<bf16_t>((const bf16_t*)q.in, q.ld, q.a, q.b, o1, q.scale, q.accumulate, rpc, direct, b % nbx, b / nbx, red);
+    else colsum_stage1<float>((const float*)q.in, q.ld, q.a, q.b, o1, q.scale, q.accumulate, rpc, direct, b % nbx, b / nbx, red);
+}
+__global__ __launch_bounds__(256) void finish_stage2_kernel(FinTable t) {
+    const int j = fin_find_job(t);
+    const FinJob& q = t.job[j];
+    colsum_stage2(q.ws, q.chunks, q.b, q.out, q.scale, q.accumulate, (int)blockIdx.x - t.blk[j]);
 }
 
 __device__ __forceinline__ float& f4e(float4& v, int c) { return reinterpret_cast<float*>(&v)[c]; }
@@ -479,6 +502,75 @@
     return 0;
 }
 
+namespace {
+constexpr int FM = ALM_FINISH_META;
+inline bool fin_meta_ok(const int* m) {
+    if (m[0] == FIN_COLSUM_F32 || m[0] == FIN_COLSUM_BF16) return m[1] >= 1 && m[2] >= 1 && m[3] >= m[2];
+    if (m[0] != FIN_SLAB) return false;
+    return m[1] >= 1 && m[2] >= 1 && m[3] >= m[2] && m[6] >= m[2] && m[6] % m[2] == 0 && m[8] >= 1 && m[9] >= 1 && (long long)m[7] >= (long long)m[6] * m[8] &&
+           m[10] >= 0 && m[11] >= 0;
+}
+inline long long fin_job_ws(const int* m) {
+    if (m[0] == FIN_SLAB) return 0;
+    const int chunks = alm_colsum_chunks(m[1]);
+    return chunks > 1 ? (long long)chunks * m[2] : 0;
+}
+}
+
+extern "C" int alm_finish_batched_ws_floats(const int* meta, int njobs) {
+    if (njobs < 0 || (njobs > 0 && !meta)) return -1;
+    long long total = 0;
+    for (int j = 0; j < njobs; ++j) {
+        if (!fin_meta_ok(meta + (long long)j * FM)) return -1;
+        total += fin_job_ws(meta + (long long)j * FM);
+    }
+    return total > 0x7fffffffLL ? -1 : (int)total;
+}
+
+extern "C" int alm_finish_batched(const void* const* ins, float* const* outs, const int* meta, int njobs, float* ws, long long ws_floats, void* stream) {
+    if (njobs <= 0) return 0;
+    if (!ins || !outs || !meta) return ALM_ERR_BAD_ARG;
+    const int need = alm_finish_batched_ws_floats(meta, njobs);
+    if (need < 0 || need > ws_floats || (need > 0 && !ws)) return ALM_ERR_BAD_ARG;
+    for (int j = 0; j < njobs; ++j)
+        if (!ins[j] || !outs[j]) return ALM_ERR_BAD_ARG;
+    long long ws_at = 0;
+    for (int j0 = 0; j0 < njobs; j0 += FIN_MAX) {
+        FinTable t1{}, t2{};
+        const int n = min(FIN_MAX, njobs - j0);
+        t1.n = t2.n = n;
+        long long g1 = 0, g2 = 0;
+        for (int j = 0; j < n; ++j) {
+            const int* m = meta + (long long)(j0 + j) * FM;
+            FinJob& q = t1.job[j];
+            q.in = ins[j0 + j]; q.out = outs[j0 + j]; q.ws = nullptr;
+            q.kind = m[0]; q.a = m[1]; q.b = m[2]; q.ld = m[3]; q.accumulate = m[4] != 0;
+            memcpy(&q.scale, &m[5], 4);
+            t1.blk[j] = (int)g1; t2.blk[j] = (int)g2;
+            if (q.kind == FIN_SLAB) {
+                q.mn = m[6]; q.slice_stride = m[7]; q.nb = m[8]; q.nb2 = m[9]; q.sC1 = m[10]; q.sC = m[11];
+                q.chunks = (q.mn + 255) / 256 < 2048 ? (q.mn + 255) / 256 : 2048;
+                g1 += (long long)q.chunks * q.nb;
+            } else {
+                q.chunks = alm_colsum_chunks(q.a);
+                g1 += (long long)((q.b + 63) / 64) * q.chunks;
+                if (q.chunks > 1) {
+                    q.ws = ws + ws_at;
+                    ws_at += (long long)q.chunks * q.b;
+                    g2 += (q.b + 255) / 256;
+                }
+            }
+            t2.job[j] = q;
+            if (g1 > 0x7fffffffLL) return ALM_ERR_UNSUPPORTED;
+        }
+        t1.blk[n] = (int)g1; t2.blk[n] = (int)g2;
+        hipLaunchKernelGGL(finish_stage1_kernel, dim3((unsigned)g1), dim3(256), 0, (hipStream_t)stream, t1);
+        if (g2 > 0) hipLaunchKernelGGL(finish_stage2_kernel, dim3((unsigned)g2), dim3(256), 0, (hipStream_t)stream, t2);
+    }
+    ALM_LAUNCH_CHECK();
+    return 0;
+}
+
 extern "C" int alm_geglu_partial_blocks(int rows) { return min(rows, 1024); }
 
 extern "C" int alm_geglu_ln_fwd(const void* u, long long ldu, int gate_offset, const float* gamma, void* out, long long ldo, float* mean,
diff --git a/audiolm-pytorch_amd/csrc/reduce.hpp b/audiolm-pytorch_amd/csrc/reduce.hpp
--- /dev/null
+++ b/audiolm-pytorch_amd/csrc/reduce.hpp
@@ -0,0 +1,77 @@
+#pragma once
+#include "common.hpp"
+
+__device__ __forceinline__ float red_scale(float v, float scale) {
+#pragma clang fp contract(off)
+    return v * scale;
+}
+__device__ __forceinline__ float red_scale_acc(const float* old, float v, float scale, int accumulate) {
+#pragma clang fp contract(off)
+    const float p = v * scale;
+    return accumulate ? *old + p : p;
+}
+
+template <typename T>
+__device__ __forceinline__ void colsum_stage1(const T* __restrict__ in, long long ld, int rows, int cols, float* __restrict__ out, float scale,
+                                              int accumulate, int rows_per_chunk, int direct, int bx, int by, float (*red)[64]) {
+    const int cx = threadIdx.x & 63, ry = threadIdx.x >> 6;
+    const int c = bx * 64 + cx;
+    const int r0 = by * rows_per_chunk, r1 = min(rows, r0 + rows_per_chunk);
+    float s0 = 0.f, s1 = 0.f, s2 = 0.f, s3 = 0.f;
+    auto ldv = [&](int r) -> float {
+        if constexpr (sizeof(T) == 2) return bf2f(in[(long long)r * ld + c]);
+        else return in[(long long)r * ld + c];
+    };
+    if (c < cols) {
+        int r = r0 + ry;
+        for (; r + 12 < r1; r += 16) {
+            s0 += ldv(r); s1 += ldv(r + 4); s2 += ldv(r + 8); s3 += ldv(r + 12);
+        }
+        for (; r < r1; r += 4) s0 += ldv(r);
+    }
+    red[ry][cx] = (s0 + s1) + (s2 + s3);
+    __syncthreads();
+    if (ry == 0 && c < cols) {
+        const float v = (red[0][cx] + red[1][cx]) + (red[2][cx] + red[3][cx]);
+        if (direct) out[c] = red_scale_acc(out + c, v, scale, accumulate);
+        else out[(long long)by * cols + c] = v;
+    }
+}
+
+__device__ __forceinline__ void colsum_stage2(const float* __restrict__ ws, int chunks, int cols, float* __restrict__ out, float scale, int accumulate, int bx) {
+    const int c = bx * 256 + threadIdx.x;
+    if (c >= cols) return;
+    float v = 0.f;
+    for (int k = 0; k < chunks; ++k) v += ws[(long long)k * cols + c];
+    out[c] = red_scale_acc(out + c, v, scale, accumulate);
+}
+
+__device__ __forceinline__ void slab_reduce(const float* __restrict__ ws, int splits, long long mn, long long slice_stride, int N, float* __restrict__ C,
+                                            long long ldc, float scale, int accumulate, int bx, int nbx) {
+#pragma clang fp contract(off)
+    const bool vec = (N & 3) == 0 && (ldc & 3) == 0 && ((uintptr_t)C & 15) == 0 && (mn & 3) == 0 && (slice_stride & 3) == 0;
+    if (vec) {
+        const long long mn4 = mn >> 2;
+        for (long long i = (long long)bx * 256 + threadIdx.x; i < mn4; i += (long long)nbx * 256) {
+            float4 s = make_float4(0.f, 0.f, 0.f, 0.f);
+            for (int z = 0; z < splits; ++z) {
+                const float4 v = *reinterpret_cast<const float4*>(ws + (long long)z * slice_stride + i * 4);
+                s.x += v.x; s.y += v.y; s.z += v.z; s.w += v.w;
+            }
+            if (scale != 1.f) { s.x = red_scale(s.x, scale); s.y = red_scale(s.y, scale); s.z = red_scale(s.z, scale); s.w = red_scale(s.w, scale); }
+            const long long e = i * 4, m = e / N, n = e % N;
+            float4* c = reinterpret_cast<float4*>(C + m * ldc + n);
+            if (accumulate) { const float4 w = *c; s.x += w.x; s.y += w.y; s.z += w.z; s.w += w.w; }
+            *c = s;
+        }
+        return;
+    }
+    for (long long i = (long long)bx * 256 + threadIdx.x; i < mn; i += (long long)nbx * 256) {
+        float s = 0.f;
+        for (int z = 0; z < splits; ++z) s += ws[(long long)z * slice_stride + i];
+        if (scale != 1.f) s = red_scale(s, scale);
+        const long long m = i / N, n = i % N;
+        float* c = C + m * ldc + n;
+        *c = accumulate ? *c + s : s;
+    }
+}
diff --git a/audiolm-pytorch_amd/launchlist.py b/audiolm-pytorch_amd/launchlist.py
--- a/audiolm-pytorch_amd/launchlist.py
+++ b/audiolm-pytorch_amd/launchlist.py
@@ -251,7 +251,7 @@
 
 def _switches(core):
     return (core.QKV_GROUP, core.QKV_GROUP_MAX_M, core.ASYNC_KV, core.DEFER_WGRAD, core.DEFER_GROUPS, core.DEFER_GROUP_SIZES, core.DEFER_MAX_BYTES, core.HC_BATCH_FINISH,
-            core.PACK_ALL, core.ASYNC_WGRAD, core.SIDE_STREAMS, ops.NT_WS)
+            core.PACK_ALL, core.ASYNC_WGRAD, core.SIDE_STREAMS, ops.NT_WS, ops.FINISH_BATCHED)
 
 
 def plan_for(core, x, mask_u8, cfg, need, bias, nflat, defer, dx_scale):
diff --git a/audiolm-pytorch_amd/ops.py b/audiolm-pytorch_amd/ops.py
--- a/audiolm-pytorch_amd/ops.py
+++ b/audiolm-pytorch_amd/ops.py
@@ -2,6 +2,7 @@
 
 import ctypes
 import os
+import struct
 
 import torch
 
@@ -163,7 +164,7 @@
     return _splitk('alm_gemm_bf16_tn_splitk', At, Bt, C, M, N, K, nb, sA, 0, sC, alpha, accumulate)
 
 
-def gemm_tn_batched(At, Bt, C, *, alpha=1.0, accumulate=False):
+def gemm_tn_batched(At, Bt, C, *, alpha=1.0, accumulate=False, finish=None):
     _chk(At, BF16), _chk(Bt, BF16), _chk(C, F32)
     assert At.dim() == 4 and Bt.dim() == 4 and C.dim() == 4 and At.stride(-1) == 1 and Bt.stride(-1) == 1 and C.stride(-1) == 1
     n1, n2, K, M = At.shape
@@ -174,7 +175,13 @@
     if nws < 0:
         raise _lib.AlmError('split-K workspace exceeds 2^31 floats')
     ws = _new(nws, dtype=F32, device=At.device) if nws > 0 else None
-    _lib.call('alm_gemm_bf16_tn_batched', At.data_ptr(), Bt.data_ptr(), C.data_ptr(), _p(ws), M, N, K, At.stride(-2), Bt.stride(-2), C.stride(-2), n1, n2,
+    name = 'alm_gemm_bf16_tn_batched'
+    if finish is not None and finish.slabs and ws is not None:
+        r = (ctypes.c_longlong * 10)()
+        if _lib.query('alm_gemm_tn_batched_reduce', M, N, K, n1, n2, C.stride(-2), C.stride(0), C.stride(1), ctypes.cast(r, ctypes.c_void_p)) and \
+                finish.slab(ws, C, list(r), accumulate):
+            name = 'alm_gemm_bf16_tn_batched_partial'
+    _lib.call(name, At.data_ptr(), Bt.data_ptr(), C.data_ptr(), _p(ws), M, N, K, At.stride(-2), Bt.stride(-2), C.stride(-2), n1, n2,
               At.stride(0), At.stride(1), sb[0], sb[1], C.stride(0), C.stride(1), float(alpha), int(accumulate), _st())
     return C
 
@@ -240,7 +247,49 @@
     return out
 
 
-def layernorm_bwd(dy, x, mean, rstd, gamma, *, extra=None, dx_dtype=F32, want_dgamma=True):
+FINISH_BATCHED = int(os.environ.get('ALM_FINISH_BATCHED', '1'))
+FIN_META = 12
+_I32 = 0x7fffffff
+
+
+class FinishList:
+
+    def __init__(self, slabs=True):
+        self.jobs = []
+        self.slabs = slabs
+
+    def __len__(self):
+        return len(self.jobs)
+
+    def colsum(self, part, out, scale=1.0, accumulate=False):
+        _chk(part), _chk(out, F32)
+        rows, cols, ld = _rows_ld(part)
+        assert part.dtype in (F32, BF16) and out.shape == (cols,) and out.is_contiguous() and rows >= 1 and ld <= _I32
+        sbits = struct.unpack('<i', struct.pack('<f', float(scale)))[0]
+        self.jobs.append((part, out.data_ptr(), [int(part.dtype == BF16), rows, cols, ld, int(accumulate), sbits, 0, 0, 0, 0, 0, 0], out))
+
+    def slab(self, ws, C, r, accumulate=False):
+        if max(r[1:]) > _I32:
+            return False
+        self.jobs.append((ws, C.data_ptr() + 4 * r[0], [2, r[1], r[2], r[3], int(accumulate), 0x3f800000, r[4], r[5], r[6], r[7], r[8], r[9]], C))
+        return True
+
+    def run(self):
+        jobs, self.jobs = self.jobs, []
+        if not jobs:
+            return
+        n = len(jobs)
+        arr_i = (ctypes.c_void_p * n)(*[j[0].data_ptr() for j in jobs])
+        arr_o = (ctypes.c_void_p * n)(*[j[1] for j in jobs])
+        meta = (ctypes.c_int * (n * FIN_META))(*[v for j in jobs for v in j[2]])
+        nws = _lib.query('alm_finish_batched_ws_floats', ctypes.cast(meta, ctypes.c_void_p), n)
+        if nws < 0:
+            raise _lib.AlmError('alm_finish_batched: malformed job or workspace above 2^31 floats')
+        ws = _new(nws, dtype=F32, device=jobs[0][0].device) if nws > 0 else None
+        _lib.call('alm_finish_batched', arr_i, arr_o, meta, n, _p(ws), nws, _st())
+
+
+def layernorm_bwd(dy, x, mean, rstd, gamma, *, extra=None, dx_dtype=F32, want_dgamma=True, finish=None):
     _chk(dy), _chk(x)
     assert dy.dtype in (BF16, F32)
     rows, D, lddy = _rows_ld(dy)
@@ -252,6 +301,10 @@
     _lib.call('alm_layernorm_bwd', dy.data_ptr(), int(dy.dtype == F32), lddy, x.data_ptr(), int(x.dtype == BF16), x.stride(0), mean.data_ptr(), rstd.data_ptr(),
               gamma.data_ptr(), _p(extra), extra.stride(0) if extra is not None else 0, dx.data_ptr(), int(dx_dtype == BF16), D, _p(part),
               rows, D, _st())
+    if want_dgamma and finish is not None:
+        dg = _new(D, dtype=F32, device=dy.device)
+        finish.colsum(part, dg)
+        return dx, dg
     return dx, (colsum(part) if want_dgamma else None)
 
 
@@ -286,7 +339,7 @@
     return out, mean, rstd
 
 
-def geglu_ln_bwd(dhn, u, gamma, mean, rstd, inner, inner_pad, du_out=None):
+def geglu_ln_bwd(dhn, u, gamma, mean, rstd, inner, inner_pad, du_out=None, finish=None):
     rows, _, ldu = _rows_ld(u)
     du = _new_like(u) if du_out is None else du_out
     assert du.shape == u.shape and du.stride(0) == ldu and du.stride(1) == 1 and du.dtype == BF16
@@ -294,6 +347,10 @@
     part = _new((nblk, inner), dtype=F32, device=u.device)
     _lib.call('alm_geglu_ln_bwd', dhn.data_ptr(), dhn.stride(0), u.data_ptr(), ldu, inner_pad, gamma.data_ptr(), mean.data_ptr(), rstd.data_ptr(),
               du.data_ptr(), part.data_ptr(), rows, inner, inner_pad, _st())
+    if finish is not None:
+        dg = _new(inner, dtype=F32, device=u.device)
+        finish.colsum(part, dg)
+        return du, dg
     return du, colsum(part)
 
 
diff --git a/include/audiolm_hip.h b/include/audiolm_hip.h
--- a/include/audiolm_hip.h
+++ b/include/audiolm_hip.h
@@ -33,6 +33,10 @@
 int alm_gemm_bf16_tn_batched(const void* At, const void* Bt, float* C, float* ws, int M, int N, int K, long long lda, long long ldb, long long ldc,
                              int nb1, int nb2, long long sA1, long long sA2, long long sB1, long long sB2, long long sC1, long long sC2, float alpha,
                              int accumulate, void* stream);
+int alm_gemm_bf16_tn_batched_partial(const void* At, const void* Bt, float* C, float* ws, int M, int N, int K, long long lda, long long ldb, long long ldc,
+                                     int nb1, int nb2, long long sA1, long long sA2, long long sB1, long long sB2, long long sC1, long long sC2, float alpha,
+                                     int accumulate, void* stream);
+int alm_gemm_tn_batched_reduce(int M, int N, int K, int nb1, int nb2, long long ldc, long long sC1, long long sC2, long long* r);
 int alm_transpose_bf16(const void* src, void* dst, int rows, int cols, long long ld_src, long long ld_dst, int rows_pad, void* stream);
 int alm_transpose_bf16_batched(const void* src, void* dst, int rows, int cols, long long ld_src, long long ld_dst, int rows_pad, int nb,
                                long long bs_src, long long bs_dst, void* stream);
@@ -56,6 +60,9 @@
                void* stream);
 int alm_colsum_chunks(int rows);
 int alm_colsum_partial(const float* in, long long ld, int rows, int cols, float* ws, void* stream);
+#define ALM_FINISH_META 12
+int alm_finish_batched_ws_floats(const int* meta, int njobs);
+int alm_finish_batched(const void* const* ins, float* const* outs, const int* meta, int njobs, float* ws, long long ws_floats, void* stream);
 
 int alm_geglu_fwd(const float* x, float* y, long long rows, int inner, void* stream);
 int alm_geglu_bwd(const float* dy, const float* x, float* dx, long long rows, int inner, void* stream);
```
